# jklebes/MetropolisEngine

Hardware: AMD Instinct MI355X
Metric: MC steps/sec (chains x sweeps) at 2^20 chains, 16 params (higher is better)
Workload: dtype f64

## Files before the change

include/metropolis_engine.h:

```cpp
#ifndef METROPOLIS_ENGINE_H
#define METROPOLIS_ENGINE_H

#include <stddef.h>
#include <stdint.h>

#ifdef __cplusplus
extern "C" {
#endif

#define ME_ABI_VERSION 1

typedef struct me_engine me_engine;

typedef enum me_status {
  ME_OK = 0,
  ME_ERR_INVALID = 1,
  ME_ERR_UNSUPPORTED = 2,
  ME_ERR_HIP = 3,
  ME_ERR_NUMERIC = 4,
  ME_ERR_STATE = 5
} me_status;

typedef enum me_dtype { ME_F32 = 0, ME_F64 = 1 } me_dtype;

// ... 61 lines not shown
  const char *user_energy_name;
} me_config;

int me_abi_version(void);

int me_load_plugin(const char *path);

int me_create(const me_config *config, me_engine **out);
int me_destroy(me_engine *engine);

int me_step(me_engine *engine, int32_t n_sweeps);
typedef enum me_step_kind_t {
  ME_STEP_ALL = 0,
  ME_STEP_REAL_GROUP = 1,
  ME_STEP_COMPLEX_GROUP = 2,
  ME_STEP_COMPLEX_MAGNITUDE_PHASE = 3
} me_step_kind_t;
int me_step_kind(me_engine *engine, int32_t kind, int32_t n_sweeps);
int me_measure(me_engine *engine);
int me_cycle(me_engine *engine, int32_t n_sweeps);
int me_cycle_stats(me_engine *engine, uint64_t *fused_cycles);
int me_set_reject_condition(me_engine *engine, int32_t reject_kind, double reject_bound);
int me_set_energy(me_engine *engine, int32_t energy_kind, const double *energy_coeffs, int32_t n_energy_coeffs,
                  const char *user_energy_name);
int me_step_injected(me_engine *engine, int32_t kind, int32_t n_sweeps, const double *normals, const double *uniforms);

int me_field_components(me_engine *engine, int32_t field, int32_t *n_components);
int me_energy_terms(me_engine *engine, int32_t *n_terms);
int me_get(me_engine *engine, int32_t field, int64_t chain_begin, int64_t n_chains, double *dst);
int me_set(me_engine *engine, int32_t field, int64_t chain_begin, int64_t n_chains, const double *src);
int me_recompute_energy(me_engine *engine);

int me_constants(me_engine *engine, double *alpha, int32_t *m, double *ratio);
int me_counters(me_engine *engine, uint64_t *step_index, uint64_t *measure_step_counter);
int me_set_counters(me_engine *engine, uint64_t step_index, uint64_t measure_step_counter);
int me_accept_stats(me_engine *engine, uint64_t *accepted, uint64_t *proposed);
int me_set_accept_stats(me_engine *engine, uint64_t accepted, uint64_t proposed);

int me_pooled_moments_size(me_engine *engine, int64_t *n_doubles);
int me_pooled_moments_geometry(me_engine *engine, int32_t *matrix_core, int32_t *tile_chains, int32_t *partial_rows);
int me_pooled_moments(me_engine *engine, double *host_out, int64_t n_doubles);
int me_pooled_moments_device(me_engine *engine, void *device_out, int64_t n_doubles);
int me_pooled_moments_begin(me_engine *engine);
int me_pooled_moments_end(me_engine *engine, double *host_out, int64_t n_doubles);
#define ME_COMM_ID_BYTES 128
int me_comm_unique_id(void *id_out, size_t bytes);
int me_comm_init_rank(me_engine *engine, const void *unique_id, size_t bytes, int32_t rank, int32_t world);
int me_comm_destroy(me_engine *engine);
int me_comm_info(me_engine *engine, int32_t *rank, int32_t *world, int32_t *rccl_version);
int me_pooled_moments_allreduce(me_engine *engine, double *host_out, int64_t n_doubles);
int me_pooled_moments_allreduce_begin(me_engine *engine);
int me_set_shared_factor(me_engine *engine, const double *packed_factor, int64_t n_doubles);
int me_set_cache_budget(int64_t bytes);
int me_get_shared_factor(me_engine *engine, double *packed_factor, int64_t n_doubles, int32_t *is_set);

int me_trace_enable(me_engine *engine, int64_t n_traced, int64_t stride);
int me_trace_shape(me_engine *engine, int64_t *rows, int64_t *cols, int64_t *n_traced);
int me_trace_get(me_engine *engine, double *dst, int64_t n_doubles);

int me_sync(me_engine *engine);
int me_set_stream(me_engine *engine, void *hip_stream);
int me_time_steps(me_engine *engine, int32_t n_launches, int32_t n_sweeps, float *elapsed_ms);

int me_set_temperature_ladder(me_engine *engine, const double *temps, int32_t n_rungs);
int me_temperature_ladder(me_engine *engine, double *temps, int32_t capacity, int32_t *n_rungs);
int me_replica_exchange(me_engine *engine, int32_t n_rounds);
int me_replica_stats(me_engine *engine, uint64_t *round, uint64_t *attempted, uint64_t *accepted, int32_t n_pairs);
int me_set_replica_stats(me_engine *engine, uint64_t round, const uint64_t *attempted, const uint64_t *accepted,
                         int32_t n_pairs);
int me_pooled_moments_range(me_engine *engine, int64_t chain_begin, int64_t n_chains, double *host_out, int64_t n_doubles);

int me_set_temperature(me_engine *engine, double temp);
int me_population_resample(me_engine *engine, double new_temp);
int me_population_stats(me_engine *engine, uint64_t *stages, double *stage_temps, double *log_weight, double *neff_fraction,
                        int64_t *n_finite, int64_t capacity);
int me_set_population_stats(me_engine *engine, uint64_t stages, const double *stage_temps, const double *log_weight,
                            const double *neff_fraction, const int64_t *n_finite);
int me_population_families(me_engine *engine, int64_t chain_begin, int64_t n, int64_t *dst);
int me_set_population_families(me_engine *engine, int64_t chain_begin, int64_t n, const int64_t *src);

int me_energy_samples_enable(me_engine *engine, int64_t capacity_records);
int me_energy_samples_record(me_engine *engine);
int me_energy_samples_count(me_engine *engine, int64_t *records, int64_t *capacity);
int me_energy_samples_get(me_engine *engine, int64_t record_begin, int64_t n_records, double *dst);
int me_energy_samples_set(me_engine *engine, int64_t n_records, const double *src);
int me_mbar_solve(me_engine *engine, double tolerance, int32_t max_iterations, double *f_out, int32_t *iterations,
                  double *residual, int64_t *n_used_out);
int me_mbar_solve_newton(me_engine *engine, double tolerance, int32_t max_iterations, double *f_out, int32_t *iterations,
                         double *residual, double *gradient, int32_t *newton_steps, int32_t *fallback_steps, int64_t *n_used_out);
int me_mbar_solve_newton_samples(int32_t device_id, const double *energies, const int32_t *rungs, int64_t n_samples,
                                 const double *ladder_temps, int32_t n_rungs, double tolerance, int32_t max_iterations,
                                 double *f_out, int32_t *iterations, double *residual, double *gradient, int32_t *newton_steps,
                                 int32_t *fallback_steps, int64_t *n_used_out);
int me_mbar_reweight(me_engine *engine, const double *f, const double *temps, int32_t n, double *ln_z, double *mean_e,
                     double *var_e, double *neff_fraction);
int me_mbar_solve_samples(int32_t device_id, const double *energies, const int32_t *rungs, int64_t n_samples,
                          const double *ladder_temps, int32_t n_rungs, double tolerance, int32_t max_iterations, double *f_out,
                          int32_t *iterations, double *residual, int64_t *n_used_out);
int me_mbar_reweight_samples(int32_t device_id, const double *energies, const int32_t *rungs, int64_t n_samples,
                             const double *ladder_temps, int32_t n_rungs, const double *f, const double *temps, int32_t n,
                             double *ln_z, double *mean_e, double *var_e, double *neff_fraction);
int me_mbar_gram(me_engine *engine, const double *f, const double *temps, int32_t n_targets, double *gram,
                 double *column_counts, double *ln_z, double *mean_e, int64_t *n_used);
int me_mbar_gram_samples(int32_t device_id, const double *energies, const int32_t *rungs, int64_t n_samples,
                         const double *ladder_temps, int32_t n_rungs, const double *f, const double *temps, int32_t n_targets,
                         double *gram, double *column_counts, double *ln_z, double *mean_e, int64_t *n_used);
// ... 71 lines not shown
```

metropolisengine_amd/_capi.py:

```python
import ctypes
import os

PKG_DIR = os.path.dirname(os.path.abspath(__file__))
LIB_PATH = os.environ.get("METROPOLIS_HIP_LIB") or os.path.join(PKG_DIR, "lib", "libmetropolis_hip.so")
ABI_VERSION = 1

ME_OK, ME_ERR_INVALID, ME_ERR_UNSUPPORTED, ME_ERR_HIP, ME_ERR_NUMERIC, ME_ERR_STATE = range(6)
ME_F32, ME_F64 = 0, 1
(ENERGY_ISO_QUAD, ENERGY_DIAG_QUAD, ENERGY_DENSE_QUAD, ENERGY_LANDAU_TOY, ENERGY_CYLINDER, ENERGY_USER,
 ENERGY_USER_INDIRECT, ENERGY_LANDAU_TERMS) = range(8)
FLAG_TRACK_COVARIANCE = 1
FLAG_REFERENCE_ENERGY_LEDGERS = 2
REJECT_NONE, REJECT_ABS_REAL0_GE, REJECT_USER = 0, 1, 2
STEP_ALL, STEP_REAL_GROUP, STEP_COMPLEX_GROUP, STEP_COMPLEX_MAGNITUDE_PHASE = range(4)
COV_REFERENCE, COV_FIXED, COV_POOLED = 0, 1, 2
COMM_ID_BYTES = 128
(FIELD_PARAMS, FIELD_ENERGY, FIELD_WIDTH, FIELD_MEAN, FIELD_COV, FIELD_OBS_MEAN, FIELD_FACTOR, FIELD_ENERGY_TOTAL) = range(8)

_dp = ctypes.POINTER(ctypes.c_double)


def double_ptr(arr):
    return arr.ctypes.data_as(_dp)

# ... 15 lines not shown
        ("temp", ctypes.c_double), ("target_acceptance", ctypes.c_double), ("sampling_width", ctypes.c_double),
        ("energy_kind", ctypes.c_int32), ("n_energy_coeffs", ctypes.c_int32), ("energy_coeffs", _dp),
        ("reject_kind", ctypes.c_int32), ("flags", ctypes.c_int32), ("reject_bound", ctypes.c_double),
        ("initial_params", _dp), ("covariance_real", _dp), ("covariance_complex", _dp),
        ("user_energy_name", ctypes.c_char_p),
    ]


_H = ctypes.c_void_p
SYMBOLS = {
    "me_abi_version": (ctypes.c_int, []),
    "me_load_plugin": (ctypes.c_int, [ctypes.c_char_p]),
    "me_create": (ctypes.c_int, [ctypes.POINTER(MeConfig), ctypes.POINTER(_H)]),
    "me_destroy": (ctypes.c_int, [_H]),
    "me_step": (ctypes.c_int, [_H, ctypes.c_int32]),
    "me_measure": (ctypes.c_int, [_H]),
    "me_cycle": (ctypes.c_int, [_H, ctypes.c_int32]),
    "me_cycle_stats": (ctypes.c_int, [_H, ctypes.POINTER(ctypes.c_uint64)]),
    "me_step_kind": (ctypes.c_int, [_H, ctypes.c_int32, ctypes.c_int32]),
    "me_set_reject_condition": (ctypes.c_int, [_H, ctypes.c_int32, ctypes.c_double]),
    "me_set_energy": (ctypes.c_int, [_H, ctypes.c_int32, _dp, ctypes.c_int32, ctypes.c_char_p]),
    "me_step_injected": (ctypes.c_int, [_H, ctypes.c_int32, ctypes.c_int32, _dp, _dp]),
    "me_field_components": (ctypes.c_int, [_H, ctypes.c_int32, ctypes.POINTER(ctypes.c_int32)]),
    "me_energy_terms": (ctypes.c_int, [_H, ctypes.POINTER(ctypes.c_int32)]),
    "me_pooled_moments_begin": (ctypes.c_int, [_H]),
    "me_pooled_moments_end": (ctypes.c_int, [_H, ctypes.POINTER(ctypes.c_double), ctypes.c_int64]),
    "me_detect_equilibration": (ctypes.c_int, [ctypes.c_int32, ctypes.POINTER(ctypes.c_double), ctypes.c_int64,
                                               ctypes.c_int64, ctypes.c_int32, ctypes.c_int32,
                                               ctypes.POINTER(ctypes.c_int64), ctypes.POINTER(ctypes.c_double),
                                               ctypes.POINTER(ctypes.c_double)]),
    "me_get": (ctypes.c_int, [_H, ctypes.c_int32, ctypes.c_int64, ctypes.c_int64, _dp]),
    "me_set": (ctypes.c_int, [_H, ctypes.c_int32, ctypes.c_int64, ctypes.c_int64, _dp]),
    "me_recompute_energy": (ctypes.c_int, [_H]),
    "me_constants": (ctypes.c_int, [_H, _dp, ctypes.POINTER(ctypes.c_int32), _dp]),
    "me_counters": (ctypes.c_int, [_H, ctypes.POINTER(ctypes.c_uint64), ctypes.POINTER(ctypes.c_uint64)]),
    "me_set_counters": (ctypes.c_int, [_H, ctypes.c_uint64, ctypes.c_uint64]),
    "me_accept_stats": (ctypes.c_int, [_H, ctypes.POINTER(ctypes.c_uint64), ctypes.POINTER(ctypes.c_uint64)]),
    "me_pooled_moments_size": (ctypes.c_int, [_H, ctypes.POINTER(ctypes.c_int64)]),
    "me_pooled_moments_geometry": (ctypes.c_int, [_H, ctypes.POINTER(ctypes.c_int32), ctypes.POINTER(ctypes.c_int32),
                                                  ctypes.POINTER(ctypes.c_int32)]),
    "me_pooled_moments": (ctypes.c_int, [_H, _dp, ctypes.c_int64]),
    "me_pooled_moments_device": (ctypes.c_int, [_H, ctypes.c_void_p, ctypes.c_int64]),
    "me_comm_unique_id": (ctypes.c_int, [ctypes.c_void_p, ctypes.c_size_t]),
    "me_comm_init_rank": (ctypes.c_int, [_H, ctypes.c_void_p, ctypes.c_size_t, ctypes.c_int32, ctypes.c_int32]),
    "me_comm_destroy": (ctypes.c_int, [_H]),
    "me_comm_info": (ctypes.c_int, [_H, ctypes.POINTER(ctypes.c_int32), ctypes.POINTER(ctypes.c_int32),
                                    ctypes.POINTER(ctypes.c_int32)]),
    "me_pooled_moments_allreduce": (ctypes.c_int, [_H, _dp, ctypes.c_int64]),
    "me_pooled_moments_allreduce_begin": (ctypes.c_int, [_H]),
    "me_set_shared_factor": (ctypes.c_int, [_H, _dp, ctypes.c_int64]),
    "me_get_shared_factor": (ctypes.c_int, [_H, _dp, ctypes.c_int64, ctypes.POINTER(ctypes.c_int32)]),
    "me_set_accept_stats": (ctypes.c_int, [_H, ctypes.c_uint64, ctypes.c_uint64]),
    "me_set_cache_budget": (ctypes.c_int, [ctypes.c_int64]),
    "me_trace_enable": (ctypes.c_int, [_H, ctypes.c_int64, ctypes.c_int64]),
    "me_trace_shape": (ctypes.c_int, [_H, ctypes.POINTER(ctypes.c_int64), ctypes.POINTER(ctypes.c_int64),
                                      ctypes.POINTER(ctypes.c_int64)]),
    "me_trace_get": (ctypes.c_int, [_H, _dp, ctypes.c_int64]),
    "me_sync": (ctypes.c_int, [_H]),
    "me_set_stream": (ctypes.c_int, [_H, ctypes.c_void_p]),
    "me_time_steps": (ctypes.c_int, [_H, ctypes.c_int32, ctypes.c_int32, ctypes.POINTER(ctypes.c_float)]),
    "me_last_error": (ctypes.c_int, [_H, ctypes.c_char_p, ctypes.c_size_t]),
    "me_supported": (ctypes.c_int, [ctypes.c_int32, ctypes.c_int32, ctypes.c_int32, ctypes.c_int32]),
    "me_set_temperature_ladder": (ctypes.c_int, [_H, _dp, ctypes.c_int32]),
    "me_temperature_ladder": (ctypes.c_int, [_H, _dp, ctypes.c_int32, ctypes.POINTER(ctypes.c_int32)]),
    "me_replica_exchange": (ctypes.c_int, [_H, ctypes.c_int32]),
    "me_replica_stats": (ctypes.c_int, [_H, ctypes.POINTER(ctypes.c_uint64), ctypes.POINTER(ctypes.c_uint64),
                                        ctypes.POINTER(ctypes.c_uint64), ctypes.c_int32]),
    "me_set_replica_stats": (ctypes.c_int, [_H, ctypes.c_uint64, ctypes.POINTER(ctypes.c_uint64),
                                            ctypes.POINTER(ctypes.c_uint64), ctypes.c_int32]),
    "me_pooled_moments_range": (ctypes.c_int, [_H, ctypes.c_int64, ctypes.c_int64, _dp, ctypes.c_int64]),
    "me_set_temperature": (ctypes.c_int, [_H, ctypes.c_double]),
    "me_population_resample": (ctypes.c_int, [_H, ctypes.c_double]),
    "me_population_stats": (ctypes.c_int, [_H, ctypes.POINTER(ctypes.c_uint64), _dp, _dp, _dp, ctypes.POINTER(ctypes.c_int64),
                                           ctypes.c_int64]),
    "me_set_population_stats": (ctypes.c_int, [_H, ctypes.c_uint64, _dp, _dp, _dp, ctypes.POINTER(ctypes.c_int64)]),
    "me_population_families": (ctypes.c_int, [_H, ctypes.c_int64, ctypes.c_int64, ctypes.POINTER(ctypes.c_int64)]),
    "me_set_population_families": (ctypes.c_int, [_H, ctypes.c_int64, ctypes.c_int64, ctypes.POINTER(ctypes.c_int64)]),
    "me_energy_samples_enable": (ctypes.c_int, [_H, ctypes.c_int64]),
    "me_energy_samples_record": (ctypes.c_int, [_H]),
    "me_energy_samples_count": (ctypes.c_int, [_H, ctypes.POINTER(ctypes.c_int64), ctypes.POINTER(ctypes.c_int64)]),
    "me_energy_samples_get": (ctypes.c_int, [_H, ctypes.c_int64, ctypes.c_int64, _dp]),
    "me_energy_samples_set": (ctypes.c_int, [_H, ctypes.c_int64, _dp]),
    "me_mbar_solve": (ctypes.c_int, [_H, ctypes.c_double, ctypes.c_int32, _dp, ctypes.POINTER(ctypes.c_int32), _dp,
                                     ctypes.POINTER(ctypes.c_int64)]),
    "me_mbar_solve_newton": (ctypes.c_int, [_H, ctypes.c_double, ctypes.c_int32, _dp, ctypes.POINTER(ctypes.c_int32), _dp, _dp,
                                            ctypes.POINTER(ctypes.c_int32), ctypes.POINTER(ctypes.c_int32),
                                            ctypes.POINTER(ctypes.c_int64)]),
    "me_mbar_solve_newton_samples": (ctypes.c_int, [ctypes.c_int32, _dp, ctypes.POINTER(ctypes.c_int32), ctypes.c_int64, _dp,
                                                    ctypes.c_int32, ctypes.c_double, ctypes.c_int32, _dp,
                                                    ctypes.POINTER(ctypes.c_int32), _dp, _dp, ctypes.POINTER(ctypes.c_int32),
                                                    ctypes.POINTER(ctypes.c_int32), ctypes.POINTER(ctypes.c_int64)]),
    "me_mbar_reweight": (ctypes.c_int, [_H, _dp, _dp, ctypes.c_int32, _dp, _dp, _dp, _dp]),
    "me_mbar_solve_samples": (ctypes.c_int, [ctypes.c_int32, _dp, ctypes.POINTER(ctypes.c_int32), ctypes.c_int64, _dp,
                                             ctypes.c_int32, ctypes.c_double, ctypes.c_int32, _dp,
                                             ctypes.POINTER(ctypes.c_int32), _dp, ctypes.POINTER(ctypes.c_int64)]),
    "me_mbar_reweight_samples": (ctypes.c_int, [ctypes.c_int32, _dp, ctypes.POINTER(ctypes.c_int32), ctypes.c_int64, _dp,
                                                ctypes.c_int32, _dp, _dp, ctypes.c_int32, _dp, _dp, _dp, _dp]),
    "me_mbar_gram": (ctypes.c_int, [_H, _dp, _dp, ctypes.c_int32, _dp, _dp, _dp, _dp, ctypes.POINTER(ctypes.c_int64)]),
    "me_mbar_gram_samples": (ctypes.c_int, [ctypes.c_int32, _dp, ctypes.POINTER(ctypes.c_int32), ctypes.c_int64, _dp,
                                            ctypes.c_int32, _dp, _dp, ctypes.c_int32, _dp, _dp, _dp, _dp,
                                            ctypes.POINTER(ctypes.c_int64)]),
    "me_mbar_energy_shift": (ctypes.c_int, [_H, _dp]),
    "me_mbar_gram_observables": (ctypes.c_int, [_H, _dp, _dp, ctypes.c_int32, _dp, _dp, _dp, _dp, _dp,
                                                ctypes.POINTER(ctypes.c_int64)]),
    "me_mbar_gram_observables_samples": (ctypes.c_int, [ctypes.c_int32, _dp, ctypes.POINTER(ctypes.c_int32), ctypes.c_int64, _dp,
                                                        ctypes.c_int32, _dp, ctypes.c_int32, _dp, _dp, ctypes.c_int32, _dp, _dp,
# ... 92 lines not shown
```

metropolisengine_amd/csrc/me_api.hip:

```cpp
#include <algorithm>
#include <cmath>
#include <cstdlib>
#include <cstring>
#include <dlfcn.h>
#include <mutex>
#include <memory>
#include <string>
#include <atomic>
#include <chrono>
#include <vector>

#include "me_engine.h"

namespace me {

static std::vector<const KernelSet *> &registry() {
  static std::vector<const KernelSet *> sets;
  return sets;
}
static std::mutex &registry_mutex() {
  static std::mutex m;
  return m;
}
void register_kernel_set(const KernelSet *set) {
// ... 80 lines not shown
static bool initial_shape_is_identity(const me_config *c) {
  if (c->covariance_real)
    for (int i = 0; i < c->n_real; ++i)
      for (int j = 0; j <= i; ++j)
        if (c->covariance_real[i * c->n_real + j] != (i == j ? 1.0 : 0.0)) return false;
  if (c->covariance_complex)
    for (int i = 0; i < c->n_complex; ++i)
      for (int j = 0; j <= i; ++j) {
        const double re = c->covariance_complex[2 * (i * c->n_complex + j)], im = c->covariance_complex[2 * (i * c->n_complex + j) + 1];
        if (re != (i == j ? 1.0 : 0.0) || (i != j && im != 0.0)) return false;
      }
  return true;
}

int fail(me_engine *e, int code, const std::string &msg) {
  if (e) e->err = msg;
  else g_create_error = msg;
  return code;
}

static void to_device_type(const double *src, size_t count, int dtype, std::vector<unsigned char> &out) {
  out.resize(count * (dtype == ME_F32 ? 4 : 8));
  if (dtype == ME_F32) {
    float *o = reinterpret_cast<float *>(out.data());
    for (size_t i = 0; i < count; ++i) o[i] = (float)src[i];
  } else {
    std::memcpy(out.data(), src, count * 8);
  }
}

hipError_t upload(DeviceBuffer &dst, const double *src, size_t count, int dtype) {
  std::vector<unsigned char> bytes;
  to_device_type(src, count, dtype, bytes);
  const hipError_t err = dst.resize(bytes.size());
  return err != hipSuccess ? err : hipMemcpy(dst.get(), bytes.data(), bytes.size(), hipMemcpyHostToDevice);
}

int refuse_stale_total(me_engine *e, const char *subject) {
  if (!e->stale_total) return ME_OK;
  return fail(e, ME_ERR_UNSUPPORTED, std::string(subject) + " not available with ME_FLAG_REFERENCE_ENERGY_LEDGERS: its two ledgers "
                                                            "make the energy of a chain ambiguous");
}

static int report_status(me_engine *e, unsigned int bits) {
  if (!bits) return ME_OK;
  ME_HIP(e, hipMemsetAsync(e->status.get(), 0, sizeof(unsigned int), e->stream));
  std::string msg = "numeric failure in at least one chain:";
  if (bits & ST_NONFINITE_ENERGY) msg += " non-finite energy;";
  if (bits & ST_BAD_PIVOT) msg += " non-positive Cholesky pivot (proposal covariance not positive definite);";
  if (bits & ST_BAD_WIDTH) msg += " sampling width <= 0;";
  return fail(e, ME_ERR_NUMERIC, msg);
}
int check_status(me_engine *e) {
  unsigned long long *scratch = e->host_scratch.get<unsigned long long>();
  ME_HIP(e, hipMemcpyAsync(&scratch[0], e->status.get(), sizeof(unsigned int), hipMemcpyDeviceToHost, e->stream));
  ME_HIP(e, hipStreamSynchronize(e->stream));
  return report_status(e, (unsigned int)scratch[0]);
}

}

using namespace me;

namespace {

int broadcast(me_engine *e, DeviceBuffer &dst, const std::vector<double> &row, bool tiled = false) {
  std::vector<unsigned char> bytes;
  to_device_type(row.data(), row.size(), e->dtype, bytes);
  ME_HIP(e, hipMemcpyAsync(e->row_dev.get(), bytes.data(), bytes.size(), hipMemcpyHostToDevice, e->stream));
  if (tiled) ME_HIP(e, launch_broadcast_tiled(dst.get(), e->row_dev.get(), (int)row.size(), e->n, e->dtype, e->stream));
  else ME_HIP(e, launch_broadcast_rows(dst.get(), e->row_dev.get(), (int)row.size(), e->n, e->dtype, e->stream));
  ME_HIP(e, hipStreamSynchronize(e->stream));
  return ME_OK;
}

template <typename T>
void gather_rows(const T *t, int comps, int64_t n_chains, double *dst) {
  for (int r = 0; r < comps; ++r)
    for (int64_t c = 0; c < n_chains; ++c) dst[c * comps + r] = (double)t[(size_t)r * n_chains + c];
}
template <typename T>
void scatter_rows(T *t, int comps, int64_t n_chains, const double *src) {
  for (int r = 0; r < comps; ++r)
    for (int64_t c = 0; c < n_chains; ++c) t[(size_t)r * n_chains + c] = (T)src[c * comps + r];
}
template <typename T>
void transpose_tiled(T *t, int entries, int64_t tile0, int64_t chain_begin, int64_t n_chains, double *dst, const double *src) {
  const size_t tile_values = (size_t)entries * 64;
  auto at = [&](int64_t c, int k) { return (size_t)((c >> 6) - tile0) * tile_values + (size_t)k * 64 + (size_t)(c & 63); };
  for (int64_t i = 0; i < n_chains; ++i)
    for (int k = 0; k < entries; ++k) {
      if (dst) dst[i * entries + k] = (double)t[at(chain_begin + i, k)];
      else t[at(chain_begin + i, k)] = (T)src[i * entries + k];
    }
}

int copy_tiled(me_engine *e, void *field_ptr, int entries, int64_t chain_begin, int64_t n_chains, double *dst, const double *src) {
  const int64_t tile0 = chain_begin >> 6, tile1 = (chain_begin + n_chains - 1) >> 6;
  const size_t tile_values = (size_t)entries * 64, n_values = (size_t)(tile1 - tile0 + 1) * tile_values;
  unsigned char *dev = (unsigned char *)field_ptr + (size_t)tile0 * tile_values * e->esize;
  std::vector<unsigned char> tmp(n_values * e->esize);
  const bool whole = (chain_begin & 63) == 0 && (((chain_begin + n_chains) & 63) == 0 || chain_begin + n_chains == e->n);
  if (dst || !whole) {
    ME_HIP(e, hipMemcpyAsync(tmp.data(), dev, tmp.size(), hipMemcpyDeviceToHost, e->stream));
    ME_HIP(e, hipStreamSynchronize(e->stream));
  }
  if (e->dtype == ME_F32) transpose_tiled(reinterpret_cast<float *>(tmp.data()), entries, tile0, chain_begin, n_chains, dst, src);
  else transpose_tiled(reinterpret_cast<double *>(tmp.data()), entries, tile0, chain_begin, n_chains, dst, src);
  if (src) {
    ME_HIP(e, hipMemcpyAsync(dev, tmp.data(), tmp.size(), hipMemcpyHostToDevice, e->stream));
    ME_HIP(e, hipStreamSynchronize(e->stream));
  }
  return dst ? check_status(e) : ME_OK;
}

int field_info(me_engine *e, int field, void **ptr, int *comps) {
  switch (field) {
    case ME_FIELD_PARAMS: *ptr = e->x.get(); *comps = e->d; return ME_OK;
    case ME_FIELD_ENERGY: *ptr = e->energy.get(); *comps = e->n_terms; return ME_OK;
    case ME_FIELD_WIDTH: *ptr = e->width.get(); *comps = e->width_rows; return ME_OK;
    case ME_FIELD_MEAN: *ptr = e->mean.get(); *comps = e->d; return ME_OK;
    case ME_FIELD_OBS_MEAN: *ptr = e->obs_mean.get(); *comps = e->nobs; return ME_OK;
    case ME_FIELD_COV:
      if (!e->cov)
        return fail(e, ME_ERR_UNSUPPORTED, "this engine keeps no per-chain covariance: for large parameter spaces it is "
                                           "kept on request only (me_config.flags: ME_FLAG_TRACK_COVARIANCE), and not "
                                           "at all where the field would pass 4 GiB");
      *ptr = e->cov.get(); *comps = e->p; return ME_OK;
    case ME_FIELD_ENERGY_TOTAL:
      if (!e->stale_total)
        return fail(e, ME_ERR_UNSUPPORTED, "this engine keeps one coherent energy ledger (sum ME_FIELD_ENERGY); a separate "
                                           "energy_total exists with ME_FLAG_REFERENCE_ENERGY_LEDGERS only");
      *ptr = e->energy.get<unsigned char>() + (size_t)e->n_terms * (size_t)e->n * e->esize; *comps = 1; return ME_OK;
    case ME_FIELD_FACTOR:
      if (!e->factor) return fail(e, ME_ERR_UNSUPPORTED, "this engine keeps no per-chain proposal factors (dimensions "
                                                         "without per-chain kernels, or a field beyond 4 GiB)");
      *ptr = e->factor.get(); *comps = e->p; return ME_OK;
    default: return fail(e, ME_ERR_INVALID, "unknown field id");
  }
}

int upload_shared_factor(me_engine *e, const double *packed) {
  ME_HIP(e, upload(e->shared_factor, packed, (size_t)e->p, e->dtype));
  if (e->shared_full) {
    std::vector<double> full((size_t)e->nr * e->nr, 0.0);
    for (int i = 0; i < e->nr; ++i)
      for (int j = 0; j <= i; ++j) full[(size_t)i * e->nr + j] = packed[i * (i + 1) / 2 + j];
    ME_HIP(e, upload(e->shared_full, full.data(), full.size(), e->dtype));
    if (e->shared_image) ME_HIP(e, e->ks->prepare_matrix(e->shared_full.get(), e->shared_image.get(), e->stream));
  }
  return ME_OK;
}

void fill_step_launch(me_engine *e, StepLaunch &l, int n_sweeps) {
  l.n_real = e->nr;
  l.n_complex = e->nc;
  l.x = e->x.get();
  l.energy = e->energy.get();
  l.width = e->width.get();
  l.factor = e->cov_kind == CK_PER_CHAIN ? e->factor.get() : e->shared_factor.get();
  l.factor_full = e->shared_full.get();
  l.factor_image = e->shared_image.get();
  l.energy_image = e->energy_image.get();
  l.coef_device = e->coef_dev.get();
  l.coef_host = e->coef.data();
  l.n_coef = (int)e->coef.size();
  l.inj_normals = nullptr;
  l.inj_uniforms = nullptr;
  l.group = GROUP_ALL;
  l.split_widths = (e->width_rows == 3 && !e->widths_synced) ? 1 : 0;
  l.stale_total = e->stale_total ? 1 : 0;
  l.cov = e->cov.get();
  l.accept_slots = e->accept_slots.get<unsigned long long>();
  l.status = e->status.get<unsigned int>();
  l.n = e->n;
  l.chain_offset = e->chain_offset;
  l.step_index = e->step_index;
  l.seed = e->seed;
  l.n_sweeps = n_sweeps;
  l.energy_kind = e->energy_kind;
  l.cov_kind = e->cov_kind;
  l.reject_kind = e->reject_kind;
  l.grid_blocks = e->grid_blocks;
  l.reject_bound = e->reject_bound;
  l.temp = e->temp;
  l.ratio = e->ratio;
  l.target_acceptance = e->target_acceptance;
  l.damping = std::max((double)e->measure_count / (double)e->m, 200.0);
  l.ladder = e->ladder.n_rungs ? e->ladder.table.get() : nullptr;
  l.tiles_per_rung = e->ladder.n_rungs ? (int)(e->n / (64ll * e->ladder.n_rungs)) : 0;
}

int check_reject_kind(me_engine *e, int reject_kind, int energy_kind, int n_real) {
  if (reject_kind < ME_REJECT_NONE || reject_kind > ME_REJECT_USER) return fail(e, ME_ERR_INVALID, "unknown reject_kind");
  if (reject_kind == ME_REJECT_USER && !is_user_kind(energy_kind))
    return fail(e, ME_ERR_INVALID, "ME_REJECT_USER needs a user-energy plugin (it supplies me_user_reject)");
  if (reject_kind == ME_REJECT_ABS_REAL0_GE && n_real == 0)
    return fail(e, ME_ERR_INVALID, "ME_REJECT_ABS_REAL0_GE needs a real parameter");
  return ME_OK;
}
int check_user_reject(me_engine *e, int reject_kind, const KernelSet *ks) {
  if (reject_kind == ME_REJECT_USER && !ks->has_user_reject)
    return fail(e, ME_ERR_UNSUPPORTED,
                "ME_REJECT_USER: this user-energy plugin defines no me_user_reject (#define ME_USER_HAS_REJECT in its source)");
  return ME_OK;
}

}

namespace me {
namespace {
std::atomic<long long> g_cache_budget{224ll << 20};
}
long long cache_budget_bytes() { return g_cache_budget.load(std::memory_order_relaxed); }
void set_cache_budget_bytes(long long bytes) { g_cache_budget.store(bytes, std::memory_order_relaxed); }
}


int me_set_cache_budget(int64_t bytes) {
  if (bytes < 0) return fail(nullptr, ME_ERR_INVALID, "cache budget must be >= 0");
  me::set_cache_budget_bytes(bytes);
  return ME_OK;
}

int me_abi_version(void) { return ME_ABI_VERSION; }

int me_supported(int32_t dtype, int32_t n_real, int32_t n_complex, int32_t energy_kind) {
  return find_kernel_set(dtype, n_real, n_complex, energy_kind, nullptr) ? 1 : 0;
}

namespace {

int validate_config(const me_config *c, const KernelSet **ks_out) {
  if (c->abi_version != ME_ABI_VERSION) return fail(nullptr, ME_ERR_INVALID, "me_config.abi_version mismatch");
  if (c->n_real < 0 || c->n_complex < 0 || c->n_real + c->n_complex == 0)
    return fail(nullptr, ME_ERR_INVALID,
                "must give at least one real or complex parameter (metropolis_engine.py:37-39)");
  if (c->n_chains <= 0) return fail(nullptr, ME_ERR_INVALID, "n_chains must be positive");
  if (!(c->temp >= 0)) return fail(nullptr, ME_ERR_INVALID, "temp must be >= 0 (metropolis_engine.py:92)");
  if (!(c->target_acceptance > 0 && c->target_acceptance < 1))
    return fail(nullptr, ME_ERR_INVALID, "target_acceptance must be in (0, 1)");
  if (!(c->sampling_width > 0)) return fail(nullptr, ME_ERR_INVALID, "sampling_width must be > 0");
  if (c->dtype != ME_F32 && c->dtype != ME_F64) return fail(nullptr, ME_ERR_INVALID, "unknown dtype");
// ... 71 lines not shown
                  "engines or use ME_COV_FIXED / ME_COV_POOLED");
    l.keep_per_chain = false;
  }
  const long long rows = std::max<long long>(c->n_real + 2 * c->n_complex, 2 * c->n_real + c->n_complex);
  if (rows * padded * esz >= limit)
    return fail(nullptr, ME_ERR_UNSUPPORTED,
                "a per-chain field would exceed 4 GiB on this engine; shard the chains over more engines");
  l.keep_cov = l.keep_per_chain ||
               ((!ks->per_chain_cov || ks->streams_packed) && ks->tracks_cov && (c->flags & ME_FLAG_TRACK_COVARIANCE));
  l.x_tiled = ks->tiled_state;
  l.width_rows = (c->n_real > 0 && c->n_complex > 0) ? 3 : 1;
  return ME_OK;
}

std::unique_ptr<me_engine> configure(const me_config *c, const KernelSet *ks, const Layout &l) {
  std::unique_ptr<me_engine> e(new me_engine);
  e->device = c->device_id;
  e->ks = ks;
  e->n_terms = ks->energy_terms(c->energy_kind);
  e->dtype = c->dtype;
  e->esize = c->dtype == ME_F32 ? 4 : 8;
  e->n = c->n_chains;
  e->nr = c->n_real;
  e->nc = c->n_complex;
  e->d = e->nr + 2 * e->nc;
  e->p = packed_total(e->nr, e->nc);
  e->nobs = n_observables(e->nr, e->nc);
  e->chain_offset = c->chain_offset;
  e->seed = c->seed;
  e->temp = c->temp;
  e->target_acceptance = c->target_acceptance;
  e->energy_kind = c->energy_kind;
  e->reject_kind = c->reject_kind;
  e->reject_bound = c->reject_bound;
  e->cov_mode = c->cov_mode;
  e->coef.assign(c->energy_coeffs, c->energy_coeffs + c->n_energy_coeffs);
  e->alpha = -norm_ppf(c->target_acceptance / 2.0);
  e->m = e->nr + e->nc;
  e->ratio = (1.0 - 1.0 / e->m) * std::sqrt(2.0 * M_PI) * std::exp(e->alpha * e->alpha / 2.0) / 2.0 * e->alpha +
             1.0 / (e->m * c->target_acceptance * (1.0 - c->target_acceptance));
  if (const char *g = std::getenv("ME_GRID_BLOCKS")) e->grid_blocks = std::atoi(g);
  e->x_tiled = l.x_tiled;
  e->stale_total = (c->flags & ME_FLAG_REFERENCE_ENERGY_LEDGERS) != 0;
  e->width_rows = l.width_rows;
  e->n_slots = (e->n + 31) / 32 + 8;
  return e;
}

int allocate(me_engine *e, const Layout &l) {
  const KernelSet *ks = e->ks;
  ME_HIP(e, hipSetDevice(e->device));
  ME_HIP(e, e->stream.create());
  const size_t n = (size_t)e->n, tiles = (size_t)padded_chains(e->n), es = e->esize;
  ME_HIP(e, e->x.resize((e->x_tiled ? tiles : n) * e->d * es));
  ME_HIP(e, e->energy.resize(n * (e->n_terms + (e->stale_total ? 1 : 0)) * es));
  ME_HIP(e, e->width.resize(n * e->width_rows * es));
  ME_HIP(e, e->mean.resize(n * e->d * es));
  ME_HIP(e, e->obs_mean.resize(n * e->nobs * es));
  if (l.keep_cov) ME_HIP(e, e->cov.resize(tiles * e->p * es));
  if (l.keep_per_chain) ME_HIP(e, e->factor.resize(tiles * e->p * es));
  ME_HIP(e, e->shared_factor.resize((size_t)e->p * es));
  if (e->nc == 0) ME_HIP(e, e->shared_full.resize((size_t)e->nr * e->nr * es));
  if (e->shared_full && ks->prepare_matrix) ME_HIP(e, e->shared_image.resize(ks->matrix_image_bytes));
  ME_HIP(e, e->row_dev.resize((size_t)std::max(std::max(e->d, e->p), e->nobs) * es));
  ME_HIP(e, e->accept_slots.resize((size_t)e->n_slots * sizeof(unsigned long long)));
  ME_HIP(e, e->accept_total.resize(sizeof(unsigned long long)));
  ME_HIP(e, e->status.resize(sizeof(unsigned int)));
  const size_t moments_bytes = sizeof(double) * (size_t)moments_size(e->nr, e->nc);
  ME_HIP(e, e->pool.dev.resize(moments_bytes));
  ME_HIP(e, e->host_scratch.allocate(64));
  e->host_scratch.get<unsigned long long>()[0] = e->host_scratch.get<unsigned long long>()[1] = 0;
  ME_HIP(e, e->pool.host.allocate(moments_bytes));
  if (pool_reduce_supported(e->nr, e->nc, e->dtype))
    ME_HIP(e, e->pool.partials.resize(sizeof(double) * (size_t)pool_reduce_blocks(e->n, e->nr, e->nc) *
                                      (size_t)(1 + e->d + e->nr + e->nc + e->d * (e->d + 1) / 2)));
  ME_HIP(e, hipMemsetAsync(e->accept_slots.get(), 0, e->accept_slots.bytes(), e->stream));
  ME_HIP(e, hipMemsetAsync(e->status.get(), 0, sizeof(unsigned int), e->stream));
  return ME_OK;
}

int upload_coefficients(me_engine *e) {
  const std::vector<double> &coef = e->coef;
  const bool runtime_dims = e->ks->n_real < 0;
  std::vector<double> form;
  if (runtime_dims && e->energy_kind == ME_ENERGY_DIAG_QUAD) {
    if ((int)coef.size() != e->nr + e->nc) return fail(e, ME_ERR_INVALID, "wrong number of energy coefficients for this energy kind");
    form.assign(coef.begin(), coef.end());
    form.insert(form.end(), coef.begin() + e->nr, coef.end());
  } else if (runtime_dims && e->energy_kind == ME_ENERGY_DENSE_QUAD) {
    if ((int)coef.size() != e->d * e->d) return fail(e, ME_ERR_INVALID, "wrong number of energy coefficients for this energy kind");
    form.reserve((size_t)e->d * (e->d + 1) / 2);
    for (int i = 0; i < e->d; ++i)
      for (int j = 0; j <= i; ++j)
        form.push_back(i == j ? coef[(size_t)i * e->d + i] : coef[(size_t)i * e->d + j] + coef[(size_t)j * e->d + i]);
  } else if (e->energy_kind == ME_ENERGY_DENSE_QUAD || (is_user_kind(e->energy_kind) && !coef.empty())) {
    form = coef;
  } else {
    return ME_OK;
  }
  ME_HIP(e, upload(e->coef_dev, form.data(), form.size(), e->dtype));
  if (!runtime_dims && e->energy_kind == ME_ENERGY_DENSE_QUAD && e->ks->prepare_matrix) {
    ME_HIP(e, e->energy_image.resize(e->ks->matrix_image_bytes));
    ME_HIP(e, e->ks->prepare_matrix(e->coef_dev.get(), e->energy_image.get(), e->stream));
  }
  return ME_OK;
}

int initial_state(me_engine *e, const me_config *c) {
  std::vector<double> init(c->initial_params, c->initial_params + e->d);
  std::vector<double> obs(e->nobs);
  for (int i = 0; i < e->nr; ++i) {
    obs[i] = std::fabs(init[i]);
    obs[e->nr + e->nc + i] = init[i] * init[i];
  }
  for (int j = 0; j < e->nc; ++j) obs[e->nr + j] = std::hypot(init[e->nr + j], init[e->nr + e->nc + j]);
  const int pr = packed_real(e->nr);
  std::vector<double> c0(e->p, 0.0);
  bool identity = true;
  for (int i = 0; i < e->nr; ++i)
    for (int j = 0; j <= i; ++j) {
      const double v = c->covariance_real ? c->covariance_real[i * e->nr + j] : (i == j ? 1.0 : 0.0);
      c0[i * (i + 1) / 2 + j] = v;
      identity = identity && v == (i == j ? 1.0 : 0.0);
    }
  for (int i = 0; i < e->nc; ++i) {
    for (int j = 0; j < i; ++j) {
      const double re = c->covariance_complex ? c->covariance_complex[2 * (i * e->nc + j)] : 0.0;
      const double im = c->covariance_complex ? c->covariance_complex[2 * (i * e->nc + j) + 1] : 0.0;
      c0[pr + i * i + 2 * j] = re;
      c0[pr + i * i + 2 * j + 1] = im;
      identity = identity && re == 0.0 && im == 0.0;
    }
    const double dg = c->covariance_complex ? c->covariance_complex[2 * (i * e->nc + i)] : 1.0;
    c0[pr + i * i + 2 * i] = dg;
    identity = identity && dg == 1.0;
  }
  std::vector<double> f0 = c0;
  for (int i = 0; i < e->nc; ++i)
    for (int j = 0; j < i; ++j) f0[pr + i * i + 2 * j + 1] = -f0[pr + i * i + 2 * j + 1];
  if (!host_factor(f0, e->nr, e->nc))
    return fail(e, ME_ERR_INVALID, "initial covariance matrix is not positive definite (metropolis_engine.py:270)");
  int rc = ME_OK;
  std::vector<double> width_row((size_t)e->width_rows, c->sampling_width);
  if ((rc = broadcast(e, e->x, init, e->x_tiled)) || (rc = broadcast(e, e->mean, init)) || (rc = broadcast(e, e->obs_mean, obs)) ||
      (rc = broadcast(e, e->width, width_row)) || (e->cov && (rc = broadcast(e, e->cov, c0, true))) ||
      (e->factor && (rc = broadcast(e, e->factor, f0, true))) || (rc = upload_shared_factor(e, f0.data())))
    return rc;
  e->cov_kind = identity ? CK_IDENTITY : (e->ks->n_real < 0 && e->factor) ? CK_PER_CHAIN : CK_SHARED;
  return ME_OK;
}

int initial_energy(me_engine *e) {
  const int rc = me_recompute_energy(e);
  if (rc != ME_OK) return rc;
  const hipError_t herr = hipStreamSynchronize(e->stream);
  if (herr != hipSuccess) return fail(e, ME_ERR_HIP, std::string("initial energy evaluation: ") + hipGetErrorString(herr));
  return ME_OK;
}

}

int me_create(const me_config *c, me_engine **out) {
  if (!c || !out) return fail(nullptr, ME_ERR_INVALID, "null config or output pointer");
  *out = nullptr;
  const KernelSet *ks = nullptr;
  Layout layout;
  int rc;
  if ((rc = validate_config(c, &ks)) || (rc = decide_layout(c, ks, layout))) return rc;
  int n_dev = 0;
  if (hipGetDeviceCount(&n_dev) != hipSuccess || n_dev <= 0)
    return fail(nullptr, ME_ERR_HIP, "no HIP device available (this library has no CPU fallback)");
  if (c->device_id < 0 || c->device_id >= n_dev) return fail(nullptr, ME_ERR_INVALID, "device_id out of range");

  std::unique_ptr<me_engine> e = configure(c, ks, layout);
  if ((rc = allocate(e.get(), layout)) || (rc = upload_coefficients(e.get())) || (rc = initial_state(e.get(), c)) ||
      (rc = initial_energy(e.get())))
    return fail(nullptr, rc, e->err);
  *out = e.release();
  return ME_OK;
}

int me_set_reject_condition(me_engine *e, int32_t reject_kind, double reject_bound) {
  if (!e) return ME_ERR_INVALID;
  int rc;
  if ((rc = check_reject_kind(e, reject_kind, e->energy_kind, e->nr)) || (rc = check_user_reject(e, reject_kind, e->ks))) return rc;
  e->reject_kind = reject_kind;
  e->reject_bound = reject_bound;
  return ME_OK;
}

int me_set_energy(me_engine *e, int32_t energy_kind, const double *coeffs, int32_t n_coeffs, const char *user_name) {
  if (!e) return ME_ERR_INVALID;
  if (n_coeffs < 0 || (n_coeffs > 0 && !coeffs)) return fail(e, ME_ERR_INVALID, "energy coefficients missing");
  if (e->ks->n_real < 0) return fail(e, ME_ERR_UNSUPPORTED, "me_set_energy: not available on the runtime-dimension kernel set");
  if (energy_kind == ME_ENERGY_DENSE_QUAD)
    return fail(e, ME_ERR_UNSUPPORTED, "me_set_energy: the dense quadratic form keeps device images of its matrix; create a new engine");
  const KernelSet *ks = find_kernel_set(e->dtype, e->nr, e->nc, energy_kind, user_name);
// ... 1 lines not shown
    return fail(e, ME_ERR_UNSUPPORTED, is_user_kind(energy_kind)
                    ? std::string("no user-energy plugin named '") + (user_name ? user_name : "") + "' is loaded for these dimensions"
                    : "energy kind " + std::to_string(energy_kind) + " is not compiled for these dimensions");
  if (ks->tiled_state != e->ks->tiled_state || ks->per_chain_cov != e->ks->per_chain_cov || ks->streams_packed != e->ks->streams_packed ||
      ks->tracks_cov != e->ks->tracks_cov)
    return fail(e, ME_ERR_UNSUPPORTED, "me_set_energy: the plugin was built with other per-chain covariance options than this engine's kernel set");
  if (e->reject_kind == ME_REJECT_USER && !ks->has_user_reject)
    return fail(e, ME_ERR_UNSUPPORTED, "me_set_energy: the engine's wall is the plugin's me_user_reject, which the new energy does not define");
  const int n_terms = ks->energy_terms(energy_kind);
  ME_HIP(e, hipSetDevice(e->device));
  ME_HIP(e, hipStreamSynchronize(e->stream));
  DeviceBuffer ledger, coef_dev;
  if (n_terms != e->n_terms)
    ME_HIP(e, ledger.resize((size_t)e->n * (size_t)(n_terms + (e->stale_total ? 1 : 0)) * e->esize));
  if (is_user_kind(energy_kind) && n_coeffs > 0) ME_HIP(e, upload(coef_dev, coeffs, (size_t)n_coeffs, e->dtype));
  if (n_terms != e->n_terms) {
    e->energy = std::move(ledger);
    e->n_terms = n_terms;
    if (e->trace.chains > 0) e->trace.restart();
  }
  e->coef.assign(coeffs, coeffs + n_coeffs);
  e->coef_dev = std::move(coef_dev);
  e->ks = ks;
  e->energy_kind = energy_kind;
  const int rc = me_recompute_energy(e);
  if (rc != ME_OK) return rc;
  ME_HIP(e, hipStreamSynchronize(e->stream));
  return check_status(e);
}

int me_load_plugin(const char *path) {
  if (!path) return fail(nullptr, ME_ERR_INVALID, "null plugin path");
  void *handle = dlopen(path, RTLD_NOW | RTLD_GLOBAL);
  if (!handle) return fail(nullptr, ME_ERR_INVALID, std::string("dlopen failed: ") + dlerror());
  return ME_OK;
}

int me_destroy(me_engine *e) {
  if (!e) return ME_ERR_INVALID;
  (void)hipSetDevice(e->device);
  if (e->stream) (void)hipStreamSynchronize(e->stream);
  if (e->pool.copy_stream) (void)hipStreamSynchronize(e->pool.copy_stream);
  delete e;
  return ME_OK;
}

int me_recompute_energy(me_engine *e) {
  if (!e) return ME_ERR_INVALID;
  ME_HIP(e, hipSetDevice(e->device));
  EnergyLaunch l;
  l.n_real = e->nr;
  l.n_complex = e->nc;
  l.total_row = e->stale_total ? e->n_terms : -1;
  l.x = e->x.get();
  l.energy = e->energy.get();
  l.coef_device = e->coef_dev.get();
  l.coef_host = e->coef.data();
  l.n_coef = (int)e->coef.size();
  l.status = e->status.get<unsigned int>();
  l.n = e->n;
  l.energy_kind = e->energy_kind;
  l.grid_blocks = e->grid_blocks;
  hipError_t err = e->ks->init_energy(l, e->stream);
  if (err == hipErrorInvalidValue) return fail(e, ME_ERR_INVALID, "wrong number of energy coefficients for this energy kind");
  ME_HIP(e, err);
  return ME_OK;
}

static int split_widths(me_engine *e) {
  if (e->width_rows != 3 || !e->widths_synced) return ME_OK;
  const size_t row = (size_t)e->n * e->esize;
  for (int r = 1; r <= 2; ++r)
    ME_HIP(e, hipMemcpyAsync(e->width.get<unsigned char>() + r * row, e->width.get(), row, hipMemcpyDeviceToDevice, e->stream));
  e->widths_synced = false;
  return ME_OK;
}

static int resolve_step_kind(me_engine *e, int kind, int *group, bool *magphase) {
  *magphase = false;
  *group = GROUP_ALL;
  const bool mixed = e->nr > 0 && e->nc > 0;
  switch (kind) {
    case ME_STEP_ALL: return ME_OK;
    case ME_STEP_REAL_GROUP:
      if (e->nr == 0) return fail(e, ME_ERR_INVALID, "this engine has no real parameters");
      *group = mixed ? GROUP_REAL : GROUP_ALL;
      return ME_OK;
    case ME_STEP_COMPLEX_GROUP:
      if (e->nc == 0) return fail(e, ME_ERR_INVALID, "this engine has no complex parameters");
      *group = mixed ? GROUP_COMPLEX : GROUP_ALL;
      return ME_OK;
    case ME_STEP_COMPLEX_MAGNITUDE_PHASE:
      if (e->nc == 0) return fail(e, ME_ERR_INVALID, "this engine has no complex parameters");
      if (!e->ks->magphase || !e->cov)
        return fail(e, ME_ERR_UNSUPPORTED, "the magnitude-phase sampler needs the per-chain covariance kernels");
      *magphase = true;
      return ME_OK;
    default: return fail(e, ME_ERR_INVALID, "unknown step kind");
  }
}

static void count_steps(me_engine *e, int n_sweeps, int group = GROUP_ALL, bool magphase = false) {
  if (group == GROUP_ALL && !magphase) e->widths_synced = true;
  e->step_index += (unsigned long long)n_sweeps;
  e->proposed += (unsigned long long)e->n * (unsigned long long)n_sweeps * (magphase ? 2ull : 1ull);
}

static int launch_step_kind(me_engine *e, int kind, int n_sweeps, const void *inj_normals, const void *inj_uniforms) {
  int group;
  bool magphase;
  int rc = resolve_step_kind(e, kind, &group, &magphase);
  if (rc != ME_OK) return rc;
  if ((group != GROUP_ALL || magphase) && (rc = split_widths(e)) != ME_OK) return rc;
  StepLaunch l;
  fill_step_launch(e, l, n_sweeps);
  l.group = group;
  l.inj_normals = inj_normals;
  l.inj_uniforms = inj_uniforms;
  hipError_t err = magphase ? e->ks->magphase(l, e->stream) : e->ks->step(l, e->stream);
  if (err == hipErrorNotSupported) return fail(e, ME_ERR_UNSUPPORTED, "this step kind is not compiled for this engine");
  ME_HIP(e, err);
  count_steps(e, n_sweeps, group, magphase);
  return ME_OK;
}

int me_step(me_engine *e, int32_t n_sweeps) { return me_step_kind(e, ME_STEP_ALL, n_sweeps); }

int me_step_kind(me_engine *e, int32_t kind, int32_t n_sweeps) {
  if (!e) return ME_ERR_INVALID;
  if (n_sweeps <= 0) return fail(e, ME_ERR_INVALID, "n_sweeps must be positive");
  ME_HIP(e, hipSetDevice(e->device));
  return launch_step_kind(e, kind, n_sweeps, nullptr, nullptr);
}

int me_step_injected(me_engine *e, int32_t kind, int32_t n_sweeps, const double *normals, const double *uniforms) {
  if (!e || !normals || !uniforms) return ME_ERR_INVALID;
  if (n_sweeps <= 0) return fail(e, ME_ERR_INVALID, "n_sweeps must be positive");
  if (e->dtype != ME_F64) return fail(e, ME_ERR_UNSUPPORTED, "injected-stream replay is compiled for float64 engines only");
  ME_HIP(e, hipSetDevice(e->device));
  const bool magphase = kind == ME_STEP_COMPLEX_MAGNITUDE_PHASE;
  const size_t n = (size_t)e->n, k = (size_t)n_sweeps;
  const size_t nz = magphase ? (size_t)e->nc : (size_t)e->d, nu = magphase ? (size_t)e->nc + 2 : 1;
  std::vector<double> zn(k * nz * n), un(k * nu * n);
  for (size_t s = 0; s < k; ++s)
    for (size_t c = 0; c < n; ++c) {
      for (size_t j = 0; j < nz; ++j) zn[(s * nz + j) * n + c] = normals[(s * n + c) * nz + j];
      for (size_t j = 0; j < nu; ++j) un[(s * nu + j) * n + c] = uniforms[(s * n + c) * nu + j];
    }
  DeviceBuffer zd, ud;
  ME_HIP(e, zd.resize(zn.size() * sizeof(double)));
  if (ud.resize(un.size() * sizeof(double)) != hipSuccess) return fail(e, ME_ERR_HIP, "hipMalloc of the injected uniforms failed");
  if (hipMemcpy(zd.get(), zn.data(), zd.bytes(), hipMemcpyHostToDevice) != hipSuccess ||
      hipMemcpy(ud.get(), un.data(), ud.bytes(), hipMemcpyHostToDevice) != hipSuccess)
    return fail(e, ME_ERR_HIP, "upload of the injected streams failed");
  int rc = launch_step_kind(e, kind, n_sweeps, zd.get(), ud.get());
  if (rc == ME_OK && hipStreamSynchronize(e->stream) != hipSuccess) rc = fail(e, ME_ERR_HIP, "injected step failed");
  return rc;
}

namespace {
void fill_measure_launch(me_engine *e, MeasureLaunch &l, unsigned long long count) {
  l.n_real = e->nr;
  l.n_complex = e->nc;
  l.x = e->x.get();
  l.width = e->width.get();
  l.mean = e->mean.get();
  l.cov = e->cov.get();
  l.obs_mean = e->obs_mean.get();
  l.factor = e->factor.get();
  l.status = e->status.get<unsigned int>();
  l.n = e->n;
  l.measure_count = count;
  l.update_cov = (count > 50 && e->cov) ? 1 : 0;
  l.split_widths = (e->width_rows == 3 && !e->widths_synced) ? 1 : 0;
  l.write_factor = (l.update_cov && e->cov_mode == ME_COV_REFERENCE) ? 1 : 0;
  l.grid_blocks = e->grid_blocks;
}

int commit_measure(me_engine *e, const MeasureLaunch &l) {
  e->measure_count = l.measure_count;
  if (l.write_factor) e->cov_kind = CK_PER_CHAIN;
  if (e->trace.chains > 0) {
    const long long cols = e->d + e->n_terms + e->width_rows;
    if (e->trace.rows == e->trace.capacity) {
      const long long cap = e->trace.capacity ? 2 * e->trace.capacity : 1024;
      DeviceBuffer bigger;
      ME_HIP(e, bigger.resize(sizeof(double) * (size_t)(cap * cols * e->trace.chains)));
      if (e->trace.dev) {
        ME_HIP(e, hipMemcpyAsync(bigger.get(), e->trace.dev.get(), sizeof(double) * (size_t)(e->trace.rows * cols * e->trace.chains),
                                 hipMemcpyDeviceToDevice, e->stream));
        ME_HIP(e, hipStreamSynchronize(e->stream));
      }
      e->trace.dev = std::move(bigger);
      e->trace.capacity = cap;
    }
    const int rows_valid = (e->width_rows == 3 && e->widths_synced) ? 1 : e->width_rows;
    double *row = e->trace.dev.get<double>() + e->trace.rows * cols * e->trace.chains;
    ME_HIP(e, launch_trace(e->x.get(), e->energy.get(), e->width.get(), e->n, e->d, e->n_terms, rows_valid, e->dtype, e->trace.chains,
                           e->trace.stride, row, e->stream, e->x_tiled));
    if (rows_valid != e->width_rows) {
      double *widths = row + (size_t)(e->d + e->n_terms) * e->trace.chains;
      for (int r = 1; r < 3; ++r)
        ME_HIP(e, hipMemcpyAsync(widths + (size_t)r * e->trace.chains, widths, sizeof(double) * (size_t)e->trace.chains,
                                 hipMemcpyDeviceToDevice, e->stream));
    }
    e->trace.rows += 1;
  }
  return ME_OK;
}
}

int me_measure(me_engine *e) {
  if (!e) return ME_ERR_INVALID;
  ME_HIP(e, hipSetDevice(e->device));
  MeasureLaunch l;
  fill_measure_launch(e, l, e->measure_count + 1);
  ME_HIP(e, e->ks->measure(l, e->stream));
  return commit_measure(e, l);
}

int me_cycle(me_engine *e, int32_t n_sweeps) {
  if (!e) return ME_ERR_INVALID;
  if (n_sweeps <= 0) return fail(e, ME_ERR_INVALID, "n_sweeps must be positive");
  ME_HIP(e, hipSetDevice(e->device));
  if (e->ks->cycle) {
    StepLaunch sl;
    fill_step_launch(e, sl, n_sweeps);
    MeasureLaunch ml;
    fill_measure_launch(e, ml, e->measure_count + 1);
    ml.split_widths = 0;
    const hipError_t err = e->ks->cycle(sl, ml, e->stream);
    if (err == hipSuccess) {
      count_steps(e, n_sweeps);
      e->fused_cycles += 1;
      return commit_measure(e, ml);
    }
    if (err != hipErrorNotSupported) ME_HIP(e, err);
    (void)hipGetLastError();
  }
  const int rc = me_step(e, n_sweeps);
  return rc != ME_OK ? rc : me_measure(e);
}

int me_cycle_stats(me_engine *e, uint64_t *fused_cycles) {
  if (!e || !fused_cycles) return ME_ERR_INVALID;
  *fused_cycles = e->fused_cycles;
  return ME_OK;
}

int me_trace_enable(me_engine *e, int64_t n_traced, int64_t stride) {
  if (!e) return ME_ERR_INVALID;
  if (n_traced < 0 || stride < 1 || (n_traced > 0 && (n_traced - 1) * stride >= e->n))
    return fail(e, ME_ERR_INVALID, "traced chains out of range");
  ME_HIP(e, hipSetDevice(e->device));
  ME_HIP(e, hipStreamSynchronize(e->stream));
  e->trace.restart();
  e->trace.chains = n_traced;
  e->trace.stride = stride;
  return ME_OK;
}

int me_trace_shape(me_engine *e, int64_t *rows, int64_t *cols, int64_t *n_traced) {
  if (!e) return ME_ERR_INVALID;
  if (rows) *rows = e->trace.rows;
  if (cols) *cols = e->d + e->n_terms + e->width_rows;
  if (n_traced) *n_traced = e->trace.chains;
  return ME_OK;
}

int me_trace_get(me_engine *e, double *dst, int64_t n_doubles) {
  if (!e || !dst) return ME_ERR_INVALID;
  const long long want = e->trace.rows * (e->d + e->n_terms + e->width_rows) * e->trace.chains;
  if (n_doubles != want) return fail(e, ME_ERR_INVALID, "wrong trace buffer length");
  if (want == 0) return ME_OK;
  ME_HIP(e, hipSetDevice(e->device));
  ME_HIP(e, hipStreamSynchronize(e->stream));
  ME_HIP(e, hipMemcpy(dst, e->trace.dev.get(), sizeof(double) * (size_t)want, hipMemcpyDeviceToHost));
  return ME_OK;
}

int me_field_components(me_engine *e, int32_t field, int32_t *n_components) {
  if (!e || !n_components) return ME_ERR_INVALID;
  void *ptr;
  int comps;
  int rc = field_info(e, field, &ptr, &comps);
  if (rc == ME_OK) *n_components = comps;
  return rc;
}

int me_energy_terms(me_engine *e, int32_t *n_terms) {
  if (!e || !n_terms) return ME_ERR_INVALID;
  *n_terms = e->n_terms;
  return ME_OK;
}

int me_get(me_engine *e, int32_t field, int64_t chain_begin, int64_t n_chains, double *dst) {
  if (!e || !dst) return ME_ERR_INVALID;
  if (chain_begin < 0 || n_chains < 0 || chain_begin + n_chains > e->n) return fail(e, ME_ERR_INVALID, "chain range out of bounds");
  ME_HIP(e, hipSetDevice(e->device));
  void *ptr;
  int comps;
  int rc = field_info(e, field, &ptr, &comps);
  if (rc != ME_OK) return rc;
  if (n_chains == 0) return ME_OK;
  if (field == ME_FIELD_COV || field == ME_FIELD_FACTOR || (field == ME_FIELD_PARAMS && e->x_tiled))
    return copy_tiled(e, ptr, comps, chain_begin, n_chains, dst, nullptr);
  std::vector<unsigned char> tmp((size_t)comps * n_chains * e->esize);
  for (int r = 0; r < comps; ++r)
    ME_HIP(e, hipMemcpyAsync(tmp.data() + (size_t)r * n_chains * e->esize,
                             (const unsigned char *)ptr + ((size_t)r * e->n + chain_begin) * e->esize,
                             (size_t)n_chains * e->esize, hipMemcpyDeviceToHost, e->stream));
  ME_HIP(e, hipStreamSynchronize(e->stream));
  if (e->dtype == ME_F32) gather_rows(reinterpret_cast<const float *>(tmp.data()), comps, n_chains, dst);
  else gather_rows(reinterpret_cast<const double *>(tmp.data()), comps, n_chains, dst);
  if (field == ME_FIELD_WIDTH && e->width_rows == 3 && e->widths_synced)
    for (int64_t c = 0; c < n_chains; ++c) dst[c * 3 + 1] = dst[c * 3 + 2] = dst[c * 3];
  return check_status(e);
}

int me_set(me_engine *e, int32_t field, int64_t chain_begin, int64_t n_chains, const double *src) {
  if (!e || !src) return ME_ERR_INVALID;
  if (chain_begin < 0 || n_chains < 0 || chain_begin + n_chains > e->n) return fail(e, ME_ERR_INVALID, "chain range out of bounds");
  ME_HIP(e, hipSetDevice(e->device));
  void *ptr;
  int comps;
  int rc = field_info(e, field, &ptr, &comps);
  if (rc != ME_OK) return rc;
  if (field == ME_FIELD_WIDTH && e->width_rows == 3 && (chain_begin != 0 || n_chains != e->n))
    return fail(e, ME_ERR_INVALID, "widths of a mixed engine must be set for all chains at once");
  if (n_chains == 0) return ME_OK;
  if (field == ME_FIELD_COV || field == ME_FIELD_FACTOR || (field == ME_FIELD_PARAMS && e->x_tiled)) {
    rc = copy_tiled(e, ptr, comps, chain_begin, n_chains, nullptr, src);
    if (rc != ME_OK) return rc;
    if (field == ME_FIELD_FACTOR) e->cov_kind = CK_PER_CHAIN;
    return ME_OK;
  }
  std::vector<unsigned char> tmp((size_t)comps * n_chains * e->esize);
  if (e->dtype == ME_F32) scatter_rows(reinterpret_cast<float *>(tmp.data()), comps, n_chains, src);
  else scatter_rows(reinterpret_cast<double *>(tmp.data()), comps, n_chains, src);
  for (int r = 0; r < comps; ++r)
    ME_HIP(e, hipMemcpyAsync((unsigned char *)ptr + ((size_t)r * e->n + chain_begin) * e->esize,
                             tmp.data() + (size_t)r * n_chains * e->esize, (size_t)n_chains * e->esize,
                             hipMemcpyHostToDevice, e->stream));
  ME_HIP(e, hipStreamSynchronize(e->stream));
  if (field == ME_FIELD_FACTOR) e->cov_kind = CK_PER_CHAIN;
  if (field == ME_FIELD_WIDTH && e->width_rows == 3) e->widths_synced = false;
  return ME_OK;
}

int me_constants(me_engine *e, double *alpha, int32_t *m, double *ratio) {
  if (!e) return ME_ERR_INVALID;
  if (alpha) *alpha = e->alpha;
  if (m) *m = e->m;
  if (ratio) *ratio = e->ratio;
  return ME_OK;
}

int me_counters(me_engine *e, uint64_t *step_index, uint64_t *measure_step_counter) {
  if (!e) return ME_ERR_INVALID;
  if (step_index) *step_index = e->step_index;
  if (measure_step_counter) *measure_step_counter = e->measure_count;
  return ME_OK;
}

int me_set_counters(me_engine *e, uint64_t step_index, uint64_t measure_step_counter) {
  if (!e) return ME_ERR_INVALID;
  if (measure_step_counter < 1) return fail(e, ME_ERR_INVALID, "measure_step_counter starts at 1");
  e->step_index = step_index;
  e->measure_count = measure_step_counter;
  return ME_OK;
}

int me_accept_stats(me_engine *e, uint64_t *accepted, uint64_t *proposed) {
  if (!e) return ME_ERR_INVALID;
  ME_HIP(e, hipSetDevice(e->device));
  unsigned long long *scratch = e->host_scratch.get<unsigned long long>();
  ME_HIP(e, launch_sum_slots(e->accept_slots.get<unsigned long long>(), e->n_slots, e->accept_total.get<unsigned long long>(), e->stream));
  ME_HIP(e, hipMemcpyAsync(&scratch[1], e->accept_total.get(), sizeof(unsigned long long), hipMemcpyDeviceToHost, e->stream));
  ME_HIP(e, hipMemcpyAsync(&scratch[0], e->status.get(), sizeof(unsigned int), hipMemcpyDeviceToHost, e->stream));
  ME_HIP(e, hipStreamSynchronize(e->stream));
  if (accepted) *accepted = scratch[1];
  if (proposed) *proposed = e->proposed;
  return report_status(e, (unsigned int)scratch[0]);
// ... 10 lines not shown
  e->proposed = proposed;
  return ME_OK;
}

int me_pooled_moments_size(me_engine *e, int64_t *n_doubles) {
  if (!e || !n_doubles) return ME_ERR_INVALID;
  *n_doubles = moments_size(e->nr, e->nc);
  return ME_OK;
}

int me_pooled_moments_geometry(me_engine *e, int32_t *matrix_core, int32_t *tile_chains, int32_t *partial_rows) {
  if (!e || !matrix_core || !tile_chains || !partial_rows) return ME_ERR_INVALID;
  if (!e->pool.partials) return fail(e, ME_ERR_UNSUPPORTED, "pooled moments: dimension too large for the reduction kernel");
  *matrix_core = e->ks->pool_stage1 ? 1 : 0;
  *tile_chains = e->ks->pool_stage1 ? 64 : pool_tile_chains(e->nr, e->nc, e->dtype);
  *partial_rows = pool_reduce_blocks(e->n, e->nr, e->nc);
  return ME_OK;
}

namespace {
hipError_t wait_polling(hipEvent_t ev) {
  const auto t0 = std::chrono::steady_clock::now();
  for (;;) {
    const hipError_t rc = hipEventQuery(ev);
    if (rc != hipErrorNotReady) return rc;
    if (std::chrono::steady_clock::now() - t0 > std::chrono::milliseconds(2)) return hipEventSynchronize(ev);
  }
}
hipError_t wait_polling(hipStream_t stream) {
  const auto t0 = std::chrono::steady_clock::now();
  for (;;) {
    const hipError_t rc = hipStreamQuery(stream);
    if (rc != hipErrorNotReady) return rc;
    if (std::chrono::steady_clock::now() - t0 > std::chrono::milliseconds(2)) return hipStreamSynchronize(stream);
  }
}

int check_pooled(me_engine *e, int64_t n_doubles) {
  if (n_doubles != moments_size(e->nr, e->nc)) return fail(e, ME_ERR_INVALID, "wrong pooled-moment buffer length");
  if (e->pool.pending) return fail(e, ME_ERR_STATE, "a pooled-moment reduction is in flight (me_pooled_moments_end first)");
  if (!e->pool.partials) return fail(e, ME_ERR_UNSUPPORTED, "pooled moments: dimension too large for the reduction kernel");
  ME_HIP(e, hipSetDevice(e->device));
  return ME_OK;
}
int enqueue_pool_reduce(me_engine *e, const void *x, long long n_chains, long long n_slots, double proposed, double *device_out) {
  hipError_t err = launch_pool_reduce(x, n_chains, e->nr, e->nc, e->dtype, e->accept_slots.get<unsigned long long>(), n_slots, proposed,
                                      e->pool.partials.get<double>(), device_out, e->stream, e->ks->pool_stage1, e->x_tiled);
  if (err == hipErrorInvalidValue) return fail(e, ME_ERR_UNSUPPORTED, "pooled moments: dimension too large for the reduction kernel");
  ME_HIP(e, err);
  return ME_OK;
}
int enqueue_pooled_moments(me_engine *e, double *device_out, int64_t n_doubles) {
  const int rc = check_pooled(e, n_doubles);
  return rc != ME_OK ? rc : enqueue_pool_reduce(e, e->x.get(), e->n, e->n_slots, (double)e->proposed, device_out);
}
int fetch_pooled_moments(me_engine *e, double *host_out, int64_t n_doubles) {
  const size_t bytes = sizeof(double) * (size_t)n_doubles;
  ME_HIP(e, hipMemcpyAsync(e->pool.host.get<double>(), e->pool.dev.get(), bytes, hipMemcpyDeviceToHost, e->stream));
  ME_HIP(e, wait_polling(e->stream));
  std::memcpy(host_out, e->pool.host.get<double>(), bytes);
  return ME_OK;
}
}

int me_pooled_moments_device(me_engine *e, void *device_out, int64_t n_doubles) {
  if (!e || !device_out) return ME_ERR_INVALID;
  int rc = enqueue_pooled_moments(e, (double *)device_out, n_doubles);
  if (rc != ME_OK) return rc;
  ME_HIP(e, wait_polling(e->stream));
  return ME_OK;
}

int me_pooled_moments(me_engine *e, double *host_out, int64_t n_doubles) {
  if (!e || !host_out) return ME_ERR_INVALID;
  const int rc = enqueue_pooled_moments(e, e->pool.dev.get<double>(), n_doubles);
  return rc != ME_OK ? rc : fetch_pooled_moments(e, host_out, n_doubles);
}

int me_pooled_moments_range(me_engine *e, int64_t chain_begin, int64_t n_chains, double *host_out, int64_t n_doubles) {
  if (!e || !host_out) return ME_ERR_INVALID;
  if (chain_begin < 0 || n_chains <= 0 || chain_begin + n_chains > e->n || chain_begin % 64 != 0 || n_chains % 64 != 0)
    return fail(e, ME_ERR_INVALID, "the chain range must be whole 64-chain tiles inside the engine");
  int rc = check_pooled(e, n_doubles);
  if (rc != ME_OK) return rc;
  const unsigned char *x = e->x.get<unsigned char>();
  if (e->x_tiled) {
    x += (size_t)chain_begin * e->d * e->esize;
  } else {
    const size_t row = (size_t)n_chains * e->esize;
    if (row * e->d > e->pool.range_x.bytes()) {
      ME_HIP(e, hipStreamSynchronize(e->stream));
      ME_HIP(e, e->pool.range_x.reserve(row * e->d));
    }
    ME_HIP(e, hipMemcpy2DAsync(e->pool.range_x.get(), row, x + (size_t)chain_begin * e->esize, (size_t)e->n * e->esize, row, (size_t)e->d,
                               hipMemcpyDeviceToDevice, e->stream));
    x = e->pool.range_x.get<unsigned char>();
  }
  if ((rc = enqueue_pool_reduce(e, x, n_chains, 0, 0.0, e->pool.dev.get<double>())) != ME_OK) return rc;
  return fetch_pooled_moments(e, host_out, n_doubles);
}

namespace {
int begin_pooled(me_engine *e, bool allreduce) {
  if (e->pool.pending) return fail(e, ME_ERR_STATE, "a pooled-moment reduction is already in flight: call me_pooled_moments_end first");
  if (allreduce && !e->comm)
    return fail(e, ME_ERR_STATE, "this engine has no communicator: call me_comm_init_rank first (single-GPU engines use me_pooled_moments)");
  ME_HIP(e, hipSetDevice(e->device));
  if (!e->pool.copy_stream) {
    ME_HIP(e, e->pool.copy_stream.create());
    ME_HIP(e, e->pool.reduced.create(hipEventDisableTiming));
    ME_HIP(e, e->pool.copied.create(hipEventDisableTiming));
  }
  const int64_t n_doubles = moments_size(e->nr, e->nc);
  int rc = enqueue_pooled_moments(e, e->pool.dev.get<double>(), n_doubles);
  if (rc != ME_OK) return rc;
  ME_HIP(e, hipEventRecord(e->pool.reduced, e->stream));
  ME_HIP(e, hipStreamWaitEvent(e->pool.copy_stream, e->pool.reduced, 0));
  if (allreduce) {
    const ncclResult_t nrc = e->rccl->all_reduce(e->pool.dev.get<double>(), e->pool.dev.get<double>(), (size_t)n_doubles, ncclDouble, ncclSum, e->comm, e->pool.copy_stream);
    if (nrc != ncclSuccess) return fail(e, ME_ERR_HIP, std::string("ncclAllReduce: ") + e->rccl->error_string(nrc));
  }
  ME_HIP(e, hipMemcpyAsync(e->pool.host.get<double>(), e->pool.dev.get<double>(), sizeof(double) * (size_t)n_doubles, hipMemcpyDeviceToHost, e->pool.copy_stream));
  ME_HIP(e, hipEventRecord(e->pool.copied, e->pool.copy_stream));
  e->pool.pending = true;
  return ME_OK;
}
}

int me_pooled_moments_begin(me_engine *e) {
  if (!e) return ME_ERR_INVALID;
  return begin_pooled(e, false);
}

int me_pooled_moments_allreduce_begin(me_engine *e) {
  if (!e) return ME_ERR_INVALID;
  return begin_pooled(e, true);
}

// ... 63 lines not shown
    *rccl_version = v;
  }
  return ME_OK;
}

int me_pooled_moments_end(me_engine *e, double *host_out, int64_t n_doubles) {
  if (!e || !host_out) return ME_ERR_INVALID;
  if (!e->pool.pending) return fail(e, ME_ERR_STATE, "no pooled-moment reduction in flight: call me_pooled_moments_begin first");
  if (n_doubles != moments_size(e->nr, e->nc)) return fail(e, ME_ERR_INVALID, "wrong pooled-moment buffer length");
  ME_HIP(e, hipSetDevice(e->device));
  ME_HIP(e, wait_polling(e->pool.copied));
  e->pool.pending = false;
  std::memcpy(host_out, e->pool.host.get<double>(), sizeof(double) * (size_t)n_doubles);
  return ME_OK;
}

int me_set_shared_factor(me_engine *e, const double *packed_factor, int64_t n_doubles) {
  if (!e || !packed_factor) return ME_ERR_INVALID;
  if (e->cov_mode != ME_COV_POOLED) return fail(e, ME_ERR_STATE, "me_set_shared_factor needs cov_mode = ME_COV_POOLED");
  if (n_doubles != e->p) return fail(e, ME_ERR_INVALID, "wrong packed factor length");
  ME_HIP(e, hipSetDevice(e->device));
  ME_HIP(e, hipStreamSynchronize(e->stream));
  int rc = upload_shared_factor(e, packed_factor);
  if (rc != ME_OK) return rc;
  e->cov_kind = CK_SHARED;
  e->shared_host.assign(packed_factor, packed_factor + n_doubles);
  return ME_OK;
}

int me_get_shared_factor(me_engine *e, double *packed_factor, int64_t n_doubles, int32_t *is_set) {
  if (!e || !is_set) return ME_ERR_INVALID;
  *is_set = e->shared_host.empty() ? 0 : 1;
  if (!*is_set) return ME_OK;
  if (!packed_factor || n_doubles != e->p) return fail(e, ME_ERR_INVALID, "wrong packed factor length");
  std::copy(e->shared_host.begin(), e->shared_host.end(), packed_factor);
  return ME_OK;
}

int me_sync(me_engine *e) {
  if (!e) return ME_ERR_INVALID;
  ME_HIP(e, hipSetDevice(e->device));
  ME_HIP(e, hipStreamSynchronize(e->stream));
  return check_status(e);
}

int me_set_stream(me_engine *e, void *hip_stream) {
  if (!e) return ME_ERR_INVALID;
  ME_HIP(e, hipSetDevice(e->device));
  ME_HIP(e, hipStreamSynchronize(e->stream));
  e->stream.lend((hipStream_t)hip_stream);
  return ME_OK;
}

int me_time_steps(me_engine *e, int32_t n_launches, int32_t n_sweeps, float *elapsed_ms) {
  if (!e || !elapsed_ms) return ME_ERR_INVALID;
  if (n_launches <= 0 || n_sweeps <= 0) return fail(e, ME_ERR_INVALID, "n_launches and n_sweeps must be positive");
  ME_HIP(e, hipSetDevice(e->device));
  if (!e->time_start) {
    ME_HIP(e, e->time_start.create());
    ME_HIP(e, e->time_stop.create());
  }
  hipEvent_t start = e->time_start, stop = e->time_stop;
  ME_HIP(e, hipEventRecord(start, e->stream));
  for (int i = 0; i < n_launches; ++i) {
    StepLaunch l;
    fill_step_launch(e, l, n_sweeps);
    hipError_t err = e->ks->step(l, e->stream);
    if (err != hipSuccess) return fail(e, ME_ERR_HIP, std::string("step launch: ") + hipGetErrorString(err));
    count_steps(e, n_sweeps);
  }
  ME_HIP(e, hipEventRecord(stop, e->stream));
  ME_HIP(e, hipEventSynchronize(stop));
  ME_HIP(e, hipEventElapsedTime(elapsed_ms, start, stop));
  return ME_OK;
}

int me_last_error(me_engine *e, char *buf, size_t buf_bytes) {
  if (!buf || buf_bytes == 0) return ME_ERR_INVALID;
  const std::string &s = e ? e->err : g_create_error;
  const size_t k = std::min(buf_bytes - 1, s.size());
  std::memcpy(buf, s.data(), k);
  buf[k] = 0;
  return ME_OK;
}
```

metropolisengine_amd/csrc/me_device.h:

```cpp
#pragma once

#include <type_traits>
#include <utility>

#include <hip/hip_runtime.h>
#include <stdint.h>

#include "me_internal.h"
#include "me_math64.h"

namespace me {

struct U4 {
  uint32_t x, y, z, w;
};

__device__ __forceinline__ uint32_t xor3(uint32_t a, uint32_t b, uint32_t c) {
  return __builtin_amdgcn_bitop3_b32(a, b, c, 0x96);
}
__device__ __forceinline__ U4 philox4x32_10(U4 c, uint32_t k0, uint32_t k1) {
#pragma unroll
  for (int r = 0; r < 10; ++r) {
    const uint64_t p0 = (uint64_t)0xD2511F53u * c.x;
    const uint64_t p1 = (uint64_t)0xCD9E8D57u * c.z;
    U4 n;
    n.x = xor3((uint32_t)(p1 >> 32), c.y, k0);
    n.y = (uint32_t)p1;
    n.z = xor3((uint32_t)(p0 >> 32), c.w, k1);
    n.w = (uint32_t)p0;
    c = n;
    k0 += 0x9E3779B9u;
    k1 += 0xBB67AE85u;
  }
  return c;
}
__device__ __forceinline__ U4 philox_counter(unsigned long long gid, unsigned long long step, int b) {
  U4 ctr;
  ctr.x = (uint32_t)gid;
  ctr.y = (uint32_t)(gid >> 32);
  ctr.z = (uint32_t)step;
  ctr.w = ((uint32_t)(step >> 32) << 16) | (uint32_t)b;
  return ctr;
}
__device__ __forceinline__ U4 philox_block(unsigned long long gid, unsigned long long step, int b, uint32_t seed_lo, uint32_t seed_hi) {
  return philox4x32_10(philox_counter(gid, step, b), seed_lo, seed_hi);
}

__device__ __forceinline__ float fma_(float a, float b, float c) { return __builtin_fmaf(a, b, c); }
__device__ __forceinline__ double fma_(double a, double b, double c) { return __builtin_fma(a, b, c); }

template <typename R>
struct Num;

template <>
struct Num<float> {
  static __device__ __forceinline__ void prepare() {}
  static __device__ __forceinline__ float unit(uint32_t w) {
    return __builtin_fmaf((float)w, 2.3283064365386963e-10f, 1.1641532182693481e-10f);
  }
  static __device__ __forceinline__ void normal_pair(uint32_t wa, uint32_t wb, float &g0, float &g1) {
    const float u1 = unit(wa), u2 = unit(wb);
    const float r = __builtin_amdgcn_sqrtf(-1.3862943611198906f * __builtin_amdgcn_logf(u1));
// ... 793 lines not shown
        static_for<NC>([&](auto row_index) {
          constexpr int i = decltype(row_index)::value;
          R are = 0, aim = 0;
          static_for<i>([&](auto col_index) {
            constexpr int j = decltype(col_index)::value;
            const R lre = use(std::integral_constant<int, cre(NR * (NR + 1) / 2, i, j)>{});
            const R lim = use(std::integral_constant<int, cim(NR * (NR + 1) / 2, i, j)>{});
            const R wre = g[NR + j] * R(0.70710678118654752440), wim = g[NR + NC + j] * R(0.70710678118654752440);
            are += lre * wre - lim * wim;
            aim += lre * wim + lim * wre;
          });
          const R ld = use(std::integral_constant<int, cdiag(NR * (NR + 1) / 2, i)>{});
          are += ld * (g[NR + i] * R(0.70710678118654752440));
          aim += ld * (g[NR + NC + i] * R(0.70710678118654752440));
          if constexpr (GROUP != GROUP_REAL) {
            xp[NR + i] = x[NR + i] + w_c * are;
            xp[NR + NC + i] = x[NR + NC + i] + w_c * aim;
          }
        });
        bool rejected = false;
        if (a.reject_kind == ME_REJECT_ABS_REAL0_GE) rejected = !(N_::abs_(xp[0]) < a.reject_bound);
        else if (a.reject_kind == ME_REJECT_USER) rejected = energy_reject(en, xp, 0);
        R terms_new[Ledger::T];
        const R e_new = ledger.propose(en, xp, terms_new);
        const R diff = e_new - (stale_total ? total_q5 : ledger.partial());
        bool accept = diff <= R(0);
        if constexpr (LADDER) accept = accept || uphill_at<true>(a, c, u_accept, diff);
        else if (a.temp > R(0)) accept = accept || N_::uphill(u_accept, diff, a.inv_temp, a.inv_temp_log2e);
        accept = accept && !rejected;
        bad_energy |= (!rejected && !N_::finite(e_new));
#pragma unroll
        for (int d = 0; d < D; ++d) x[d] = accept ? xp[d] : x[d];
        if (stale_total) total_q5 = accept ? e_new : total_q5;
        else ledger.commit(accept, terms_new);
        w = N_::adapt(w, accept, a.ratio, a.p, a.damping, a.up, a.down);
        if constexpr (GROUP == GROUP_ALL) w_r = w_c = w;
        else if constexpr (GROUP == GROUP_REAL) w_r = w;
        else w_c = w;
        wave_accepted += (unsigned int)__popcll(__ballot(accept));
      }
    } else {
      run_sweeps<R, NR, NC, Energy, CK, INJECT, GROUP, LADDER>(a, en, c, gid, stale_total, x, ledger, total_q5, w, w_r, w_c, fac, wave_accepted, bad_energy);
    }
    bad_width |= !(w > R(0));
#pragma unroll
    for (int d = 0; d < D; ++d) fx.store(d, xoff, x[d]);
    if (stale_total) fe.store(Ledger::T, coff, total_q5);
    else ledger.store(fe, coff);
    fw.store(MIXED ? GROUP : 0, coff, w);
  }
  publish_step(a, blockDim.x >> 6, wave_accepted, bad_energy, bad_width);
}

template <typename R, int NR, int NC, class Energy>
__global__ void __launch_bounds__(kStepThreads) k_init_energy(const R *xs, R *energy, long long n, unsigned int *status,
                                                                Energy en, int total_row) {
  constexpr int D = NR + 2 * NC;
  energy_prepare(en, 0);
  const long long stride = (long long)gridDim.x * kStepThreads;
  for (long long c = (long long)blockIdx.x * kStepThreads + threadIdx.x; c < n; c += stride) {
    R x[D];
#pragma unroll
    for (int d = 0; d < D; ++d) x[d] = xs[state_index<R, D>(c, d, n)];
    constexpr int T = term_count<Energy>::value;
    bool finite = true;
    R total = R(0);
#pragma unroll
    for (int t = 0; t < T; ++t) {
      R e;
      if constexpr (T == 1) e = en(x);
      else e = en.term(t, x);
      energy[(long long)t * n + c] = e;
      total = t == 0 ? e : total + e;
      finite = finite && Num<R>::finite(e);
    }
    if (total_row >= 0) energy[(long long)total_row * n + c] = total;
    if (!finite) atomicOr(status, (unsigned int)ST_NONFINITE_ENERGY);
  }
}

}
#include "me_packed_walk.h"
namespace me {

template <typename R>
struct MeasureArgs {
  const R *x, *width;
  R *mean, *cov, *obs_mean, *factor;
  unsigned int *status;
  long long n;
  R keep;
  R inv_i;
  R cov_keep;
  int update_cov, write_factor, split_widths;
};

template <typename R>
MeasureArgs<R> typed_measure(const MeasureLaunch &l) {
  MeasureArgs<R> a;
  a.x = (const R *)l.x;
  a.width = (const R *)l.width;
  a.mean = (R *)l.mean;
  a.cov = (R *)l.cov;
  a.obs_mean = (R *)l.obs_mean;
  a.factor = (R *)l.factor;
  a.status = l.status;
// ... 288 lines not shown
```

metropolisengine_amd/csrc/me_engine.h:

```cpp
#pragma once

#include <string>
#include <utility>
#include <vector>

#include "me_comm.h"
#include "me_internal.h"

#pragma GCC visibility push(hidden)

namespace me {


class DeviceBuffer {
 public:
  DeviceBuffer() = default;
  DeviceBuffer(DeviceBuffer &&o) noexcept : ptr_(std::exchange(o.ptr_, nullptr)), bytes_(std::exchange(o.bytes_, 0)) {}
  DeviceBuffer &operator=(DeviceBuffer &&o) noexcept {
    if (this != &o) {
      reset();
      ptr_ = std::exchange(o.ptr_, nullptr);
      bytes_ = std::exchange(o.bytes_, 0);
    }
    return *this;
  }
  ~DeviceBuffer() { reset(); }
  void reset() {
    if (ptr_) (void)hipFree(ptr_);
    ptr_ = nullptr;
    bytes_ = 0;
  }
  hipError_t resize(size_t bytes) {
    if (bytes == bytes_) return hipSuccess;
    reset();
    if (bytes == 0) return hipSuccess;
    const hipError_t err = hipMalloc(&ptr_, bytes);
    if (err == hipSuccess) bytes_ = bytes;
    else ptr_ = nullptr;
    return err;
  }
  hipError_t reserve(size_t bytes) { return bytes <= bytes_ ? hipSuccess : resize(bytes); }
  template <typename T = void>
  T *get() const { return static_cast<T *>(ptr_); }
  size_t bytes() const { return bytes_; }
  explicit operator bool() const { return ptr_ != nullptr; }

 private:
  void *ptr_ = nullptr;
  size_t bytes_ = 0;
};

class PinnedBuffer {
 public:
  PinnedBuffer() = default;
  PinnedBuffer(const PinnedBuffer &) = delete;
  PinnedBuffer &operator=(const PinnedBuffer &) = delete;
  ~PinnedBuffer() { reset(); }
  void reset() {
    if (ptr_) (void)hipHostFree(ptr_);
    ptr_ = nullptr;
// ... 25 lines not shown
    if (owned_ && stream_) (void)hipStreamDestroy(stream_);
    stream_ = theirs;
    owned_ = false;
  }
  operator hipStream_t() const { return stream_; }

 private:
  hipStream_t stream_ = nullptr;
  bool owned_ = false;
};

class Event {
 public:
  Event() = default;
  Event(const Event &) = delete;
  Event &operator=(const Event &) = delete;
  ~Event() { reset(); }
  void reset() {
    if (event_) (void)hipEventDestroy(event_);
    event_ = nullptr;
  }
  hipError_t create(unsigned flags = hipEventDefault) {
    reset();
    return hipEventCreateWithFlags(&event_, flags);
  }
  operator hipEvent_t() const { return event_; }

 private:
  hipEvent_t event_ = nullptr;
};

}

struct me_engine {
  int device = 0;
  me::Stream stream;
  const me::KernelSet *ks = nullptr;
  int dtype = ME_F32;
  size_t esize = 4;
  long long n = 0;
  int nr = 0, nc = 0, d = 0, p = 0, nobs = 0;
  unsigned long long chain_offset = 0, seed = 0;
  double temp = 0, target_acceptance = 0.3, alpha = 0, ratio = 0, reject_bound = 0;
  int m = 0, energy_kind = 0, reject_kind = 0, cov_mode = 0;
  bool stale_total = false;
  me::Event time_start, time_stop;
  std::vector<double> shared_host;
  int cov_kind = me::CK_IDENTITY;
  int grid_blocks = 0;
  int n_terms = 1;
  std::vector<double> coef;
  unsigned long long step_index = 0, measure_count = 1;
  unsigned long long fused_cycles = 0;
  me::DeviceBuffer x, energy, width, mean, cov, obs_mean;
  me::DeviceBuffer factor, shared_factor, shared_full, shared_image, energy_image, coef_dev, row_dev;
  me::DeviceBuffer accept_slots, accept_total;
  long long n_slots = 0;
  unsigned long long proposed = 0;
  bool x_tiled = false;
  int width_rows = 1;
  bool widths_synced = true;
  me::DeviceBuffer status;
  me::PinnedBuffer host_scratch;
  struct Pool {
    me::DeviceBuffer dev, partials;
    me::PinnedBuffer host;
    me::DeviceBuffer range_x;
    me::Stream copy_stream;
    me::Event reduced, copied;
    bool pending = false;
  } pool;
  const me::RcclApi *rccl = nullptr;
  ncclComm_t comm = nullptr;
  int comm_rank = 0, comm_world = 1;
  struct Trace {
    me::DeviceBuffer dev;
    long long chains = 0, stride = 1, rows = 0, capacity = 0;
    void restart() {
      dev.reset();
      rows = capacity = 0;
    }
  } trace;
  struct Ladder {
    int n_rungs = 0;
    std::vector<double> temps;
    me::DeviceBuffer table;
    me::DeviceBuffer pair_counts;
    unsigned long long round = 0;
  } ladder;
  struct Population {
    me::DeviceBuffer fam, fam_out;
    me::DeviceBuffer x, energy;
    me::DeviceBuffer anc;
    me::DeviceBuffer scratch;
    me::DeviceBuffer records;
    unsigned long long stages = 0, capacity = 0;
    std::vector<double> temps;
  } population;
  struct Samples {
    me::DeviceBuffer data;
    long long capacity = 0, rows = 0;
    me::DeviceBuffer obs;
    int n_obs = 0;
    int obs_index[ME_MAX_RECORDED_OBSERVABLES] = {};
  } samples;
  std::string err;

  ~me_engine() {
    (void)hipSetDevice(device);
    if (comm && rccl) (void)rccl->comm_destroy(comm);
  }
};

namespace me {

int fail(me_engine *e, int code, const std::string &msg);

#define ME_HIP(e, call)                                                                                      \
  do {                                                                                                       \
    hipError_t err__ = (call);                                                                               \
    if (err__ != hipSuccess)                                                                                 \
      return me::fail((e), ME_ERR_HIP, std::string(#call) + ": " + hipGetErrorString(err__));                \
  } while (0)

int check_status(me_engine *e);

hipError_t upload(DeviceBuffer &dst, const double *src, size_t count, int dtype);

int refuse_stale_total(me_engine *e, const char *subject);

inline long long padded_chains(long long n) { return (n + 63) / 64 * 64; }

}

#pragma GCC visibility pop
```

metropolisengine_amd/csrc/me_generic.hip:

```cpp
#include "me_internal.h"
#include "me_launch.h"

namespace me {
namespace {

template <typename R>
__global__ void __launch_bounds__(kBlockThreads) k_broadcast_rows(R *dst, const R *row_values, int rows, long long n) {
  const long long stride = (long long)gridDim.x * kBlockThreads;
  for (long long c = (long long)blockIdx.x * kBlockThreads + threadIdx.x; c < n; c += stride)
    for (int r = 0; r < rows; ++r) dst[(long long)r * n + c] = row_values[r];
}

template <typename R>
__global__ void __launch_bounds__(kBlockThreads) k_broadcast_tiled(R *dst, const R *entry_values, int entries, long long n_padded) {
  const long long total = n_padded * entries, stride = (long long)gridDim.x * kBlockThreads;
  for (long long i = (long long)blockIdx.x * kBlockThreads + threadIdx.x; i < total; i += stride)
    dst[i] = entry_values[(i >> 6) % entries];
}

__device__ __forceinline__ void pair_of(int p, int &i, int &j) {
  i = (int)((sqrtf(8.0f * (float)p + 1.0f) - 1.0f) * 0.5f);
  while (i * (i + 1) / 2 > p) --i;
  while ((i + 1) * (i + 2) / 2 <= p) ++i;
  j = p - i * (i + 1) / 2;
}

constexpr int kMaxEntries = 12;

template <typename R, int TILE>
__global__ void __launch_bounds__(kBlockThreads) k_pool_reduce(const R *x, long long n, int nr, int nc, int entry_base, int tiled, double *partials) {
  extern __shared__ __attribute__((aligned(16))) unsigned char smem_raw[];
  R *tile = reinterpret_cast<R *>(smem_raw);
  constexpr int kTilePitch = TILE + 1;
  const int d = nr + 2 * nc;
  const int n_aug = d + nr + nc;
  const int n_pair = d * (d + 1) / 2;
  const int n_entries = 1 + n_aug + n_pair;
  const int tid = threadIdx.x;
  auto at = [&](int r, long long c) -> long long { return tiled ? ((c >> 6) * (long long)d + r) * 64 + (c & 63) : (long long)r * n + c; };

  int row_i[kMaxEntries], row_j[kMaxEntries];
  bool active[kMaxEntries];
  double acc[kMaxEntries];
#pragma unroll
  for (int k = 0; k < kMaxEntries; ++k) {
    const int e = entry_base + tid + k * kBlockThreads;
    acc[k] = 0.0;
    row_i[k] = row_j[k] = -1;
    active[k] = e < n_entries;
    if (!active[k] || e == 0) continue;
    if (e <= n_aug) {
      row_i[k] = e - 1;
    } else {
      pair_of(e - 1 - n_aug, row_i[k], row_j[k]);
// ... 143 lines not shown
constexpr int kSumThreads = 1024;
__global__ void __launch_bounds__(kSumThreads) k_sum_slots(const unsigned long long *slots, long long n_slots,
                                                           unsigned long long *total) {
  __shared__ unsigned long long part[kSumThreads / 64];
  unsigned long long s = 0;
  long long i = threadIdx.x;
  for (; i + 7 * kSumThreads < n_slots; i += 8 * kSumThreads) {
    unsigned long long v[8];
#pragma unroll
    for (int u = 0; u < 8; ++u) v[u] = slots[i + u * kSumThreads];
#pragma unroll
    for (int u = 0; u < 8; ++u) s += v[u];
  }
  for (; i < n_slots; i += kSumThreads) s += slots[i];
#pragma unroll
  for (int w = 32; w > 0; w >>= 1) s += __shfl_xor(s, w, 64);
  if ((threadIdx.x & 63) == 0) part[threadIdx.x >> 6] = s;
  __syncthreads();
  if (threadIdx.x == 0) {
    unsigned long long t = 0;
#pragma unroll
    for (int w = 0; w < kSumThreads / 64; ++w) t += part[w];
    total[0] = t;
  }
}

template <typename R>
__global__ void __launch_bounds__(kBlockThreads) k_trace(const R *x, const R *energy, const R *width, long long n, int d,
                                                         int n_terms, int width_rows, long long n_traced, long long stride,
                                                         int tiled, double *out) {
  const long long t = (long long)blockIdx.x * kBlockThreads + threadIdx.x;
  if (t >= n_traced) return;
  const long long c = t * stride;
  for (int k = 0; k < d; ++k)
    out[(long long)k * n_traced + t] = (double)x[tiled ? ((c >> 6) * (long long)d + k) * 64 + (c & 63) : (long long)k * n + c];
  for (int k = 0; k < n_terms; ++k) out[(long long)(d + k) * n_traced + t] = (double)energy[(long long)k * n + c];
  for (int r = 0; r < width_rows; ++r)
    out[(long long)(d + n_terms + r) * n_traced + t] = (double)width[(long long)r * n + c];
}

hipError_t launch_trace(const void *x, const void *energy, const void *width, long long n, int d, int n_terms,
                        int width_rows, int dtype, long long n_traced, long long stride, double *out, hipStream_t stream,
                        bool tiled_state) {
  const dim3 grid((unsigned)((n_traced + kBlockThreads - 1) / kBlockThreads)), block(kBlockThreads);
  if (dtype == ME_F32)
    hipLaunchKernelGGL(k_trace<float>, grid, block, 0, stream, (const float *)x, (const float *)energy, (const float *)width,
                       n, d, n_terms, width_rows, n_traced, stride, tiled_state ? 1 : 0, out);
  else
    hipLaunchKernelGGL(k_trace<double>, grid, block, 0, stream, (const double *)x, (const double *)energy,
                       (const double *)width, n, d, n_terms, width_rows, n_traced, stride, tiled_state ? 1 : 0, out);
  return hipGetLastError();
}

hipError_t launch_sum_slots(const unsigned long long *slots, long long n_slots, unsigned long long *total,
                            hipStream_t stream) {
  hipLaunchKernelGGL(k_sum_slots, dim3(1), dim3(kSumThreads), 0, stream, slots, n_slots, total);
  return hipGetLastError();
}

constexpr size_t kPoolLdsLimit = 160 * 1024;
int pool_tile_chains(int nr, int nc, int dtype) {
  const int n_aug = nr + 2 * nc + nr + nc;
  const size_t elem = dtype == ME_F32 ? sizeof(float) : sizeof(double);
  for (int tile : {64, 32, 16})
    if ((size_t)n_aug * (size_t)(tile + 1) * elem <= kPoolLdsLimit) return tile;
  return 0;
}

bool pool_reduce_supported(int nr, int nc, int dtype) { return pool_tile_chains(nr, nc, dtype) != 0; }

int pool_reduce_blocks(long long n, int nr, int nc) {
  const int d = nr + 2 * nc;
  const long long n_entries = 1 + d + nr + nc + (long long)d * (d + 1) / 2;
  long long cap = (32ll << 20) / (8 * n_entries);
  if (cap > 1024) cap = 1024;
  if (cap < 64) cap = 64;
  if (d + nr + nc <= 32) cap = 256;
  const long long tiles = (n + 63) / 64;
  return (int)(tiles < cap ? (tiles < 1 ? 1 : tiles) : cap);
}

namespace {
template <typename R, int TILE>
hipError_t launch_pool_stage1(const void *x, long long n, int nr, int nc, int n_entries, int blocks, double *partials, hipStream_t stream, bool tiled) {
  const size_t lds = (size_t)(nr + 2 * nc + nr + nc) * (size_t)(TILE + 1) * sizeof(R);
  if (lds > 64 * 1024)
    if (hipError_t rc = raise_lds_limit<k_pool_reduce<R, TILE>>(kPoolLdsLimit); rc != hipSuccess) return rc;
  for (int base = 0; base < n_entries; base += kMaxEntries * kBlockThreads)
    hipLaunchKernelGGL((k_pool_reduce<R, TILE>), dim3((unsigned)blocks), dim3(kBlockThreads), lds, stream, (const R *)x, n, nr, nc, base,
                       tiled ? 1 : 0, partials);
  return hipGetLastError();
}
template <typename R>
hipError_t launch_pool_stage1_tile(int tile, const void *x, long long n, int nr, int nc, int n_entries, int blocks, double *partials, hipStream_t stream, bool tiled) {
  switch (tile) {
    case 64: return launch_pool_stage1<R, 64>(x, n, nr, nc, n_entries, blocks, partials, stream, tiled);
    case 32: return launch_pool_stage1<R, 32>(x, n, nr, nc, n_entries, blocks, partials, stream, tiled);
    case 16: return launch_pool_stage1<R, 16>(x, n, nr, nc, n_entries, blocks, partials, stream, tiled);
    default: return hipErrorInvalidValue;
  }
}
}

hipError_t launch_pool_reduce(const void *x, long long n, int nr, int nc, int dtype, const unsigned long long *slots,
                              long long n_slots, double proposed, double *partials, double *out_device,
                              hipStream_t stream,
// ... 19 lines not shown
```

metropolisengine_amd/csrc/me_internal.h:

```cpp
#pragma once

#include <hip/hip_runtime.h>
#include <stdint.h>

#include "../../include/metropolis_engine.h"

namespace me {

enum CovKind { CK_IDENTITY = 0, CK_SHARED = 1, CK_PER_CHAIN = 2, CK_PER_CHAIN_NT = 3 };

enum StepGroup { GROUP_ALL = 0, GROUP_REAL = 1, GROUP_COMPLEX = 2 };

enum StatusBits : uint32_t {
  ST_NONFINITE_ENERGY = 1u,
  ST_BAD_PIVOT = 2u,
  ST_BAD_WIDTH = 4u
};

long long cache_budget_bytes();
void set_cache_budget_bytes(long long bytes);

constexpr int kBlockThreads = 256;
#ifndef ME_STEP_THREADS
#define ME_STEP_THREADS 64
#endif
constexpr int kStepThreads = ME_STEP_THREADS;
constexpr int kFusedStepThreads = 256;
constexpr int kFusedSweepsThreshold = 4;

struct StepLaunch {
  int n_real, n_complex;
  void *x, *energy, *width;
  const void *factor;
  const void *factor_full;
  const void *factor_image;
  const void *energy_image;
  const void *coef_device;
  const double *coef_host;
  int n_coef;
  const void *inj_normals;
  const void *inj_uniforms;
  unsigned long long *accept_slots;
  unsigned int *status;
  long long n;
  unsigned long long chain_offset, step_index, seed;
  int n_sweeps, energy_kind, cov_kind, reject_kind, grid_blocks;
  int group;
  int split_widths;
  int stale_total;
  const void *cov;
  double reject_bound, temp, ratio, target_acceptance, damping;
  const void *ladder;
  int tiles_per_rung;
};

struct MeasureLaunch {
  int n_real, n_complex;
  void *x, *width, *mean, *cov, *obs_mean, *factor;
  unsigned int *status;
  long long n;
  unsigned long long measure_count;
  int update_cov;
  int split_widths;
  int write_factor;
  int grid_blocks;
};

struct EnergyLaunch {
  int n_real, n_complex;
  int total_row;
  void *x, *energy;
  const void *coef_device;
  const double *coef_host;
  int n_coef;
  unsigned int *status;
  long long n;
  int energy_kind, grid_blocks;
};

constexpr int kMaxRegisterDof = 96;

struct KernelSet {
  const char *user_name;
  int dtype, n_real, n_complex;
  bool per_chain_cov;
  bool tracks_cov;
  bool (*has_energy)(int energy_kind);
  int (*energy_terms)(int energy_kind);
  hipError_t (*step)(const StepLaunch &, hipStream_t);
  hipError_t (*magphase)(const StepLaunch &, hipStream_t);
  hipError_t (*measure)(const MeasureLaunch &, hipStream_t);
  hipError_t (*init_energy)(const EnergyLaunch &, hipStream_t);
  size_t matrix_image_bytes;
  hipError_t (*prepare_matrix)(const void *matrix, void *image, hipStream_t);
  hipError_t (*pool_stage1)(const void *x, long long n, double *partials, int n_rows, hipStream_t);
  bool has_user_reject;
  bool streams_packed;
  hipError_t (*cycle)(const StepLaunch &, const MeasureLaunch &, hipStream_t);
  bool tiled_state;
};

void register_kernel_set(const KernelSet *set);
const KernelSet *find_kernel_set(int dtype, int n_real, int n_complex, int energy_kind, const char *user_name);
bool has_dims(int dtype, int n_real, int n_complex);

hipError_t launch_broadcast_rows(void *dst, const void *row_values, int rows, long long n, int dtype,
                                 hipStream_t stream);
hipError_t launch_broadcast_tiled(void *dst, const void *entry_values, int entries, long long n, int dtype,
                                  hipStream_t stream);
hipError_t launch_pool_reduce(const void *x, long long n, int n_real, int n_complex, int dtype,
                              const unsigned long long *slots, long long n_slots, double proposed, double *partials,
                              double *out_device, hipStream_t stream,
                              hipError_t (*stage1)(const void *, long long, double *, int, hipStream_t) = nullptr,
                              bool tiled_state = false);
int pool_reduce_blocks(long long n, int n_real, int n_complex);
bool pool_reduce_supported(int n_real, int n_complex, int dtype);
int pool_tile_chains(int n_real, int n_complex, int dtype);
hipError_t launch_trace(const void *x, const void *energy, const void *width, long long n, int d, int n_terms,
                        int width_rows, int dtype, long long n_traced, long long stride, double *out, hipStream_t stream,
                        bool tiled_state = false);
hipError_t launch_sum_slots(const unsigned long long *slots, long long n_slots, unsigned long long *total,
                            hipStream_t stream);

inline int grid_for(long long n, int requested, int threads = kStepThreads) {
  long long blocks = (n + threads - 1) / threads;
  if (requested > 0 && blocks > requested) blocks = requested;
  if (blocks < 1) blocks = 1;
  return (int)blocks;
}

__host__ __device__ inline int packed_real(int nr) { return nr * (nr + 1) / 2; }
__host__ __device__ inline int packed_total(int nr, int nc) { return nr * (nr + 1) / 2 + nc * nc; }
__host__ __device__ inline int n_observables(int nr, int nc) { return 2 * nr + nc; }
__host__ __device__ inline long long moments_size(int nr, int nc) {
  const int d = nr + 2 * nc;
  return 1 + d + (long long)d * (d + 1) / 2 + n_observables(nr, nc) + 2;
}

}
```

metropolisengine_amd/csrc/me_kernels.hip:

```cpp
#include <type_traits>

#include "me_device.h"
#include "me_dense_mfma.h"
#include "me_dense_bf16x3.h"
#include "me_dense_f64.h"
#include "me_factor_tile.h"
#include "me_per_device.h"
#include "me_pool_gram.h"
#include "me_magphase.h"

#ifdef ME_USER_SOURCE
#include ME_USER_SOURCE
#endif

#ifndef ME_NR
#error "compile with -DME_NR=<n_real> -DME_NC=<n_complex>"
#endif
#ifndef ME_DENSE
#define ME_DENSE 0
#endif
#ifndef ME_PER_CHAIN
#define ME_PER_CHAIN 1
#endif
#ifndef ME_TRACK_COV
#define ME_TRACK_COV 1
#endif

namespace me {
namespace {

constexpr int NR = ME_NR;
constexpr int NC = ME_NC;
[[maybe_unused]] constexpr int D = NR + 2 * NC;
constexpr bool kLandau = (NR == 2 && NC == 1);
constexpr bool kCylinder = (NR >= 1 && NC >= 1);

#ifdef ME_USER_SOURCE
#ifdef ME_USER_N_TERMS
}
}
template <typename R>
__device__ __forceinline__ R me_user_energy(const R *x, const R *coef) {
  R s = me_user_energy_term<R>(0, x, coef);
#pragma unroll
  for (int t = 1; t < ME_USER_N_TERMS; ++t) s += me_user_energy_term<R>(t, x, coef);
  return s;
}
namespace me {
namespace {
#endif
template <typename R, int NR_, int NC_>
struct EnergyUser {
  static constexpr int D = NR_ + 2 * NC_;
  const R *coef;
  __device__ __forceinline__ R operator()(const R (&x)[D]) const { return me_user_energy<R>(x, coef); }
#ifdef ME_USER_N_TERMS
  static constexpr int kTerms = ME_USER_N_TERMS;
  static constexpr unsigned term_groups(int t) { return me_user_term_groups(t); }
  __device__ __forceinline__ R term(int t, const R (&x)[D]) const { return me_user_energy_term<R>(t, x, coef); }
#endif
#ifdef ME_USER_HAS_REJECT
  __device__ __forceinline__ bool reject(const R (&x)[D]) const { return me_user_reject<R>(x, coef); }
#endif
};
template <typename R>
using user_fn_t = R (*)(const R *, const R *);
template <typename R>
__device__ R me_user_energy_entry(const R *x, const R *coef) { return me_user_energy<R>(x, coef); }
__device__ user_fn_t<float> g_user_fn_f32 = &me_user_energy_entry<float>;
__device__ user_fn_t<double> g_user_fn_f64 = &me_user_energy_entry<double>;
template <typename R, int NR_, int NC_>
struct EnergyUserIndirect {
  static constexpr int D = NR_ + 2 * NC_;
  user_fn_t<R> fn;
  const R *coef;
  __device__ __forceinline__ R operator()(const R (&x)[D]) const { return fn(x, coef); }
#ifdef ME_USER_HAS_REJECT
  __device__ __forceinline__ bool reject(const R (&x)[D]) const { return me_user_reject<R>(x, coef); }
#endif
};
template <typename R>
user_fn_t<R> load_user_fn() {
  user_fn_t<R> fn = nullptr;
  if constexpr (std::is_same<R, float>::value) (void)hipMemcpyFromSymbol(&fn, HIP_SYMBOL(g_user_fn_f32), sizeof(fn));
  else (void)hipMemcpyFromSymbol(&fn, HIP_SYMBOL(g_user_fn_f64), sizeof(fn));
  return fn;
}
#endif

int energy_terms(int kind) {
#ifdef ME_USER_SOURCE
#ifdef ME_USER_N_TERMS
  if (kind == ME_ENERGY_USER) return ME_USER_N_TERMS;
#else
  if (kind == ME_ENERGY_USER) return 1;
#endif
  return kind == ME_ENERGY_USER_INDIRECT ? 1 : 0;
#endif
  switch (kind) {
    case ME_ENERGY_ISO_QUAD:
    case ME_ENERGY_DIAG_QUAD: return 1;
    case ME_ENERGY_DENSE_QUAD: return ME_DENSE != 0 ? 1 : 0;
    case ME_ENERGY_LANDAU_TOY: return kLandau ? 1 : 0;
    case ME_ENERGY_LANDAU_TERMS: return kLandau ? 2 : 0;
    case ME_ENERGY_CYLINDER: return kCylinder ? 1 : 0;
    default: return 0;
  }
}
bool has_energy(int kind) { return energy_terms(kind) > 0; }

template <typename R, class Energy, bool INJECT, int GROUP, bool LADDER>
hipError_t launch_step_cov(const StepLaunch &l, const StepArgs<R> &a, const Energy &en, dim3 grid, dim3 block,
                           hipStream_t stream) {
  switch (l.cov_kind) {
    case CK_IDENTITY: {
      constexpr long long state_bytes = (long long)sizeof(R) * (D + 2);
      if constexpr (!INJECT && GROUP == GROUP_ALL && !LADDER) {
        if (state_bytes * l.n > 2 * cache_budget_bytes()) {
          hipLaunchKernelGGL((k_step<R, NR, NC, Energy, CK_IDENTITY, INJECT, GROUP, true>), grid, block, 0, stream, a, en);
          break;
        }
      }
      hipLaunchKernelGGL((k_step<R, NR, NC, Energy, CK_IDENTITY, INJECT, GROUP, false, LADDER>), grid, block, 0, stream, a, en);
      break;
    }
    case CK_SHARED: hipLaunchKernelGGL((k_step<R, NR, NC, Energy, CK_SHARED, INJECT, GROUP, false, LADDER>), grid, block, 0, stream, a, en); break;
#if ME_PER_CHAIN == 2
    case CK_PER_CHAIN: {
      if constexpr (INJECT) return hipErrorInvalidValue;
      else hipLaunchKernelGGL((k_step<R, NR, NC, Energy, CK_PER_CHAIN_NT, INJECT, GROUP, false, LADDER>), grid, block, 0, stream, a, en);
      break;
    }
#elif ME_PER_CHAIN
    case CK_PER_CHAIN: {
      constexpr long long per_chain_bytes = (long long)sizeof(R) * (D + 2 + NR * (NR + 1) / 2 + NC * NC);
      if constexpr (!INJECT) {
        if (per_chain_bytes * l.n > cache_budget_bytes()) {
          hipLaunchKernelGGL((k_step<R, NR, NC, Energy, CK_PER_CHAIN_NT, INJECT, GROUP, false, LADDER>), grid, block, 0, stream, a, en);
          break;
        }
      }
      hipLaunchKernelGGL((k_step<R, NR, NC, Energy, CK_PER_CHAIN, INJECT, GROUP, false, LADDER>), grid, block, 0, stream, a, en);
      break;
    }
#endif
    default: return hipErrorInvalidValue;
  }
  return hipGetLastError();
}

template <typename R, class Energy, bool INJECT, bool LADDER = false>
hipError_t launch_step_group(const StepLaunch &l, const StepArgs<R> &a, const Energy &en, dim3 grid, dim3 block,
                             hipStream_t stream) {
  if (l.group == GROUP_ALL) return launch_step_cov<R, Energy, INJECT, GROUP_ALL, LADDER>(l, a, en, grid, block, stream);
  if constexpr (NR > 0 && NC > 0) {
    if (l.group == GROUP_REAL) return launch_step_cov<R, Energy, INJECT, GROUP_REAL, LADDER>(l, a, en, grid, block, stream);
    if (l.group == GROUP_COMPLEX) return launch_step_cov<R, Energy, INJECT, GROUP_COMPLEX, LADDER>(l, a, en, grid, block, stream);
  }
  return hipErrorInvalidValue;
}

template <typename R, class Energy>
hipError_t step_with(const StepLaunch &l, const Energy &en, hipStream_t stream) {
  const StepArgs<R> a = typed<R>(l);
  const bool per_chain = l.cov_kind == CK_PER_CHAIN;
  const int threads = (l.n_sweeps >= kFusedSweepsThreshold || (ME_PER_CHAIN == 2 && per_chain)) ? kFusedStepThreads : kStepThreads;
  const dim3 grid(grid_for(l.n, l.grid_blocks, threads)), block(threads);
  if (l.ladder) {
    if (l.inj_normals) {
// ... 244 lines not shown
#else
#define ME_SET_NAME nullptr
#endif
constexpr auto pool_stage1_f32() -> hipError_t (*)(const void *, long long, double *, int, hipStream_t) {
  if constexpr (NR == 64 && NC == 0) return launch_pool_gram64;
  else if constexpr (D + NR + NC <= 32) return launch_pool_gram32<NR, NC>;
  else return nullptr;
}
constexpr auto pool_stage1_f64() -> hipError_t (*)(const void *, long long, double *, int, hipStream_t) {
  if constexpr (NR == 64 && NC == 0) return launch_pool_gram64_f64;
  else if constexpr (D + NR + NC <= 32) return launch_pool_gram32_f64<NR, NC>;
  else return nullptr;
}
#if ME_DENSE && !defined(ME_USER_SOURCE)
hipError_t prepare_matrix_f32(const void *factor_full, void *image, hipStream_t stream) {
  if constexpr (NR == 64 && NC == 0) {
    hipLaunchKernelGGL(k_dense64_bf16_fragments<0>, dim3(1), dim3(256), 0, stream, (const float *)factor_full,
                       (unsigned int *)image);
    return hipGetLastError();
  }
  return hipSuccess;
}
[[maybe_unused]] constexpr size_t kMatrixImageBytes = (NR == 64 && NC == 0) ? sizeof(unsigned int) * kBf16FragWords : 0;
#define ME_PREPARE_MATRIX_F32 kMatrixImageBytes, (kMatrixImageBytes ? prepare_matrix_f32 : nullptr), pool_stage1_f32()
hipError_t prepare_matrix_f64(const void *matrix, void *image, hipStream_t stream) {
  if constexpr (NR == 64 && NC == 0) {
    hipLaunchKernelGGL(k_dense64_f64_fragments<0>, dim3(1), dim3(256), 0, stream, (const double *)matrix, (double *)image);
    return hipGetLastError();
  }
  return hipSuccess;
}
[[maybe_unused]] constexpr size_t kMatrixImageBytesF64 = (NR == 64 && NC == 0) ? sizeof(double) * kDense64F64ImageDoubles : 0;
#define ME_PREPARE_MATRIX_F64 kMatrixImageBytesF64, (kMatrixImageBytesF64 ? prepare_matrix_f64 : nullptr), pool_stage1_f64()
#else
#define ME_PREPARE_MATRIX_F32 0, nullptr, pool_stage1_f32()
#define ME_PREPARE_MATRIX_F64 0, nullptr, pool_stage1_f64()
#endif
#ifdef ME_USER_HAS_REJECT
constexpr bool kHasUserReject = true;
#else
constexpr bool kHasUserReject = false;
#endif
#ifndef ME_ONLY_DTYPE
#define ME_ONLY_DTYPE 0
#endif
#if ME_ONLY_DTYPE != 64
const KernelSet kSetF32 = {ME_SET_NAME, ME_F32, NR, NC, ME_PER_CHAIN != 0, (ME_PER_CHAIN != 0 || ME_TRACK_COV != 0), has_energy, energy_terms, step<float>,
                           (NC > 0 && ME_PER_CHAIN == 1) ? magphase<float> : nullptr, measure<float>, init_energy<float>,
                           ME_PREPARE_MATRIX_F32, kHasUserReject, ME_PER_CHAIN == 2, cycle<float>, D >= kTiledStateDof};
#endif
#if ME_ONLY_DTYPE != 32
const KernelSet kSetF64 = {ME_SET_NAME, ME_F64, NR, NC, ME_PER_CHAIN != 0, (ME_PER_CHAIN != 0 || ME_TRACK_COV != 0), has_energy, energy_terms, step<double>,
                           (NC > 0 && ME_PER_CHAIN == 1) ? magphase<double> : nullptr, measure<double>, init_energy<double>,
                           ME_PREPARE_MATRIX_F64, kHasUserReject, ME_PER_CHAIN == 2, cycle<double>, D >= kTiledStateDof};
#endif

struct Registrar {
  Registrar() {
#if ME_ONLY_DTYPE != 64
    register_kernel_set(&kSetF32);
#endif
#if ME_ONLY_DTYPE != 32
    register_kernel_set(&kSetF64);
#endif
  }
} registrar;

}
}
```

metropolisengine_amd/csrc/me_mbar_obs.hip:

```cpp
#include "me_mbar.h"

#pragma clang fp contract(off)

namespace me {
namespace mbar {
namespace {

constexpr int kObsTargets = 4;
constexpr int kObsCols = 4;

struct ObsSelection {
  int q[ME_MAX_RECORDED_OBSERVABLES];
};

template <typename R>
__global__ void __launch_bounds__(kThreads) k_observable_record(const R *__restrict__ x, const R *__restrict__ energy, long long n,
                                                                 int nr, int nc, int n_terms, int tiled, ObsSelection sel,
                                                                 int n_sel, double *dst) {
  const long long c = (long long)blockIdx.x * kThreads + threadIdx.x;
  if (c >= n) return;
  const int d = nr + 2 * nc, nobs = 2 * nr + nc;
  const long long x0 = tiled ? (c >> 6) * (long long)d * 64 + (c & 63) : c;
  const long long xs = tiled ? 64 : n;
  for (int j = 0; j < n_sel; ++j) {
// ... 234 lines not shown
}

int reweight_observables_common(const Source &src, const double *f, const double *temps, int n, double *mean, double *var, double *cov,
                                double *neff) {
  const int rc = check_f_and_targets(src.e, f, src.n_rungs, temps, n, 1);
  if (rc) return rc;
  Problem p;
  return mbar_check_common(src.e, p, reweight_observables(p, src, f, temps, n, mean, var, cov, neff));
}

int catalogue_size(const me_engine *e) { return e->d + e->nobs + e->n_terms; }

}

hipError_t log_denominator_enqueue(Problem &p, const MbarSamples &sm, DeviceBuffer &d) {
  const long long n_padded = tiles_of(sm.n_samples) * kTile;
  ME_MBAR_HIP(d.resize((size_t)n_padded * sizeof(double)));
  hipLaunchKernelGGL(k_mbar_log_denominator, dim3(blocks_of(sm.n_samples)), dim3(kThreads), 0, p.stream, sm.energies, sm.n_samples,
                     n_padded, p.n_rungs, p.w.table.get<const double>(), d.get<double>());
  return hipGetLastError();
}

hipError_t reweight_observables_enqueue(Problem &p, const MbarSamples &sm, const ObsColumns &oc, const double *inv_temps, int n_temps,
                                        ObsScratch &scratch, double *out) {
  hipStream_t stream = p.stream;
  const int n_blocks = blocks_of(sm.n_samples), nq_all = oc.n_columns;
  const long long n_tiles = tiles_of(sm.n_samples);
  const size_t cells = (size_t)n_temps * nq_all;
  ME_MBAR_HIP(log_denominator_enqueue(p, sm, scratch.d));
  ME_MBAR_HIP(scratch.partials.resize((size_t)n_blocks * kObsTargets * sizeof(TargetState)));
  double *o_mean = out, *o_var = o_mean + cells, *o_cov = o_var + cells, *o_neff = o_cov + cells;
  for (int t0 = 0; t0 < n_temps; t0 += kObsTargets) {
    const int nt = std::min(kObsTargets, n_temps - t0);
    for (int q0 = 0; q0 < nq_all; q0 += kObsCols) {
      const int nq = std::min(kObsCols, nq_all - q0);
      const size_t cell = (size_t)t0 * nq_all + q0;
      hipLaunchKernelGGL(k_mbar_reweight_obs, dim3(n_blocks), dim3(kThreads), 0, stream, sm.energies, scratch.d.get<const double>(),
                         oc.data + (size_t)q0 * oc.column_stride, sm.n_samples, oc.n_chains, oc.record_stride, oc.column_stride, nq,
                         inv_temps + t0, nt, n_tiles, scratch.partials.get<TargetState>());
      hipLaunchKernelGGL(k_mbar_reweight_obs_finish, dim3(nt), dim3(kThreads), 0, stream, scratch.partials.get<const TargetState>(),
                         n_blocks, nq, nq_all, p.n_used, q0 == 0 ? 1 : 0, o_mean + cell, o_var + cell, o_cov + cell, o_neff + t0);
    }
  }
  return hipGetLastError();
}

hipError_t observable_record_enqueue(me_engine *e, long long row) {
  me_engine::Samples &s = e->samples;
  ObsSelection sel;
  for (int j = 0; j < ME_MAX_RECORDED_OBSERVABLES; ++j) sel.q[j] = j < s.n_obs ? s.obs_index[j] : 0;
  double *dst = s.obs.get<double>() + (size_t)row * (size_t)s.n_obs * (size_t)e->n;
  const dim3 grid((unsigned)((e->n + kThreads - 1) / kThreads));
  if (e->dtype == ME_F32)
    hipLaunchKernelGGL(k_observable_record<float>, grid, dim3(kThreads), 0, e->stream, e->x.get<const float>(), e->energy.get<const float>(),
                       e->n, e->nr, e->nc, e->n_terms, e->x_tiled ? 1 : 0, sel, s.n_obs, dst);
  else
    hipLaunchKernelGGL(k_observable_record<double>, grid, dim3(kThreads), 0, e->stream, e->x.get<const double>(),
                       e->energy.get<const double>(), e->n, e->nr, e->nc, e->n_terms, e->x_tiled ? 1 : 0, sel, s.n_obs, dst);
  return hipGetLastError();
}

}
}

using namespace me;
using namespace me::mbar;

extern "C" {

int me_observable_samples_enable(me_engine *e, const int32_t *indices, int32_t n_observables) {
  if (!e) return ME_ERR_INVALID;
  const int rc = refuse_stale_total(e, "observable samples are");
  if (rc != ME_OK) return rc;
  if (n_observables < 0 || n_observables > ME_MAX_RECORDED_OBSERVABLES)
    return fail(e, ME_ERR_INVALID, "n_observables must lie in [0, " + std::to_string(ME_MAX_RECORDED_OBSERVABLES) + "]");
  me_engine::Samples &s = e->samples;
  ME_HIP(e, hipSetDevice(e->device));
  if (n_observables == 0) {
    ME_HIP(e, hipStreamSynchronize(e->stream));
    s.obs.reset();
    s.n_obs = 0;
    return ME_OK;
  }
  if (!s.data) return fail(e, ME_ERR_STATE, "observable samples need the energy store: call me_energy_samples_enable first");
  if (!indices) return fail(e, ME_ERR_INVALID, "indices missing");
  for (int j = 0; j < n_observables; ++j)
    if (indices[j] < 0 || indices[j] >= catalogue_size(e))
      return fail(e, ME_ERR_INVALID, "observable index " + std::to_string(indices[j]) + " outside the catalogue of " +
                                         std::to_string(catalogue_size(e)) + " quantities");
  ME_HIP(e, hipStreamSynchronize(e->stream));
  s.obs.reset();
  s.n_obs = 0;
  s.rows = 0;
  const size_t bytes = (size_t)s.capacity * (size_t)n_observables * (size_t)e->n * sizeof(double);
  ME_HIP(e, s.obs.resize(bytes));
  if (bytes) {
    ME_HIP(e, hipMemsetAsync(s.obs.get(), 0, bytes, e->stream));
    ME_HIP(e, hipStreamSynchronize(e->stream));
  }
  s.n_obs = n_observables;
  for (int j = 0; j < n_observables; ++j) s.obs_index[j] = indices[j];
  return ME_OK;
}

int me_observable_samples_info(me_engine *e, int32_t *n_observables, int32_t *indices) {
  if (!e) return ME_ERR_INVALID;
  if (n_observables) *n_observables = e->samples.n_obs;
  if (indices)
    for (int j = 0; j < e->samples.n_obs; ++j) indices[j] = e->samples.obs_index[j];
  return ME_OK;
// ... 53 lines not shown
```

metropolisengine_amd/csrc/me_population.hip:

```cpp
#include <algorithm>
#include <cmath>
#include <vector>

#include "me_device.h"
#include "me_engine.h"

namespace me {
namespace {

constexpr int kPopThreads = 256;
constexpr int kPopWaves = kPopThreads / 64;
constexpr int kPopItems = 8;
constexpr int kPopChunk = kPopThreads * kPopItems;
constexpr int kFinalThreads = 256;
constexpr long long kSerialSlots = 8;

struct PopParams {
  double M, W, u;
  long long hi;
  long long n_finite;
};

template <typename R>
__device__ __forceinline__ double chain_log_weight(const Field<R> &fe, long long c, long long n, int n_terms, double neg_dbeta,
// ... 238 lines not shown
}

template <class F>
__device__ __forceinline__ void copy_rows(const F &src, const F &dst, unsigned int src_off, unsigned int dst_off, int rows) {
  constexpr int B = 8;
  for (int r0 = 0; r0 < rows; r0 += B) {
    decltype(src.load(0, 0u)) v[B];
#pragma unroll
    for (int k = 0; k < B; ++k)
      if (r0 + k < rows) v[k] = src.load(r0 + k, src_off);
#pragma unroll
    for (int k = 0; k < B; ++k)
      if (r0 + k < rows) dst.store(r0 + k, dst_off, v[k]);
  }
}

template <typename R>
__global__ void __launch_bounds__(kPopThreads) k_pop_gather(const R *x, const R *energy, const long long *fam, R *x_out,
                                                           R *energy_out, long long *fam_out, long long n, int d, int n_terms,
                                                           int tiled, const unsigned int *ancestors, const PopParams *params) {
  const long long j = (long long)blockIdx.x * kPopThreads + threadIdx.x;
  if (j >= n) return;
  const long long hi = params->hi;
  const long long a = (long long)ancestors[j < hi ? j : hi - 1];
  const unsigned int a_off = (unsigned int)a * (unsigned int)sizeof(R), j_off = (unsigned int)j * (unsigned int)sizeof(R);
  if (tiled) copy_rows(TiledField<R>(x, n, d), TiledField<R>(x_out, n, d), tiled_offset<R>(a, d), tiled_offset<R>(j, d), d);
  else copy_rows(Field<R>(x, n, d), Field<R>(x_out, n, d), a_off, j_off, d);
  copy_rows(Field<R>(energy, n, n_terms), Field<R>(energy_out, n, n_terms), a_off, j_off, n_terms);
  fam_out[j] = fam[a];
}

__global__ void __launch_bounds__(kPopThreads) k_pop_init_families(long long *fam, long long n, unsigned long long chain_offset) {
  const long long j = (long long)blockIdx.x * kPopThreads + threadIdx.x;
  if (j < n) fam[j] = (long long)(chain_offset + (unsigned long long)j);
}

template <typename R>
hipError_t launch(me_engine *e, double neg_dbeta) {
  me_engine::Population &pop = e->population;
  const long long n = e->n;
  hipStream_t stream = e->stream;
  const int n_blocks = (int)((n + kPopChunk - 1) / kPopChunk);
  const unsigned slot_blocks = (unsigned)((n + kPopThreads - 1) / kPopThreads);
  double *partials = pop.scratch.get<double>(), *factors = partials + 4 * (size_t)n_blocks, *offsets = factors + n_blocks;
  PopParams *params = (PopParams *)(offsets + n_blocks + 1);
  double *record = pop.records.get<double>() + 3 * (size_t)pop.stages;
  hipLaunchKernelGGL(k_pop_weights<R>, dim3(n_blocks), dim3(kPopThreads), 0, stream, e->energy.get<const R>(), n, e->n_terms,
                     neg_dbeta, partials);
  hipLaunchKernelGGL(k_pop_finalize, dim3(1), dim3(kFinalThreads), 0, stream, (const double *)partials, n_blocks, n,
                     e->chain_offset, pop.stages, (uint32_t)e->seed, (uint32_t)(e->seed >> 32), factors, offsets, params, record);
  hipLaunchKernelGGL(k_pop_scan_ancestors<R>, dim3(n_blocks), dim3(kPopThreads), 0, stream, e->energy.get<const R>(), n,
                     e->n_terms, neg_dbeta, (const double *)partials, (const double *)factors, (const double *)offsets,
                     (const PopParams *)params, pop.anc.get<unsigned int>());
  hipLaunchKernelGGL(k_pop_gather<R>, dim3(slot_blocks), dim3(kPopThreads), 0, stream, e->x.get<const R>(), e->energy.get<const R>(),
                     pop.fam.get<const long long>(), pop.x.get<R>(), pop.energy.get<R>(), pop.fam_out.get<long long>(), n, e->d,
                     e->n_terms, e->x_tiled ? 1 : 0, pop.anc.get<const unsigned int>(), (const PopParams *)params);
  return hipGetLastError();
}

size_t population_scratch_doubles(long long n) {
  const long long n_blocks = (n + kPopChunk - 1) / kPopChunk;
  return (size_t)(4 * n_blocks + n_blocks + n_blocks + 1) + (sizeof(PopParams) + sizeof(double) - 1) / sizeof(double);
}

int ensure_families(me_engine *e) {
  me_engine::Population &pop = e->population;
  if (pop.fam) return ME_OK;
  ME_HIP(e, pop.fam.resize((size_t)e->n * sizeof(long long)));
  hipLaunchKernelGGL(k_pop_init_families, dim3((unsigned)((e->n + kPopThreads - 1) / kPopThreads)), dim3(kPopThreads), 0, e->stream,
                     pop.fam.get<long long>(), e->n, e->chain_offset);
  ME_HIP(e, hipGetLastError());
  return ME_OK;
}
int ensure_population_scratch(me_engine *e) {
  me_engine::Population &pop = e->population;
  const size_t energy_bytes = (size_t)e->n * (size_t)e->n_terms * e->esize;
  if (pop.energy.bytes() < energy_bytes) {
    if (pop.energy) ME_HIP(e, hipStreamSynchronize(e->stream));
    ME_HIP(e, pop.energy.reserve(energy_bytes));
  }
  if (!pop.x) {
    ME_HIP(e, pop.x.resize(e->x.bytes()));
    ME_HIP(e, hipMemcpyAsync(pop.x.get(), e->x.get(), pop.x.bytes(), hipMemcpyDeviceToDevice, e->stream));
  }
  ME_HIP(e, pop.fam_out.resize((size_t)e->n * sizeof(long long)));
  ME_HIP(e, pop.anc.resize((size_t)e->n * sizeof(unsigned int)));
  ME_HIP(e, pop.scratch.resize(population_scratch_doubles(e->n) * sizeof(double)));
  return ME_OK;
}
int ensure_records(me_engine *e, unsigned long long stages) {
  me_engine::Population &pop = e->population;
  if (stages <= pop.capacity) return ME_OK;
  unsigned long long cap = std::max<unsigned long long>(256, pop.capacity);
  while (cap < stages) cap *= 2;
  DeviceBuffer grown;
  ME_HIP(e, grown.resize((size_t)cap * 3 * sizeof(double)));
  if (pop.records) {
    ME_HIP(e, hipMemcpyAsync(grown.get(), pop.records.get(), (size_t)pop.stages * 3 * sizeof(double), hipMemcpyDeviceToDevice, e->stream));
    ME_HIP(e, hipStreamSynchronize(e->stream));
  }
  pop.records = std::move(grown);
  pop.capacity = cap;
  return ME_OK;
}
int check_family_range(me_engine *e, int64_t chain_begin, int64_t n) {
  if (chain_begin < 0 || n < 0 || chain_begin + n > e->n) return fail(e, ME_ERR_INVALID, "family range outside the engine's chains");
  return ME_OK;
}

}
}

using namespace me;

extern "C" {

int me_set_temperature(me_engine *e, double temp) {
  if (!e) return ME_ERR_INVALID;
  if (!(std::isfinite(temp) && temp >= 0)) return fail(e, ME_ERR_INVALID, "temp must be finite and >= 0");
  if (e->ladder.n_rungs) return fail(e, ME_ERR_STATE, "this engine has a temperature ladder: its rungs carry the temperatures");
  e->temp = temp;
  return ME_OK;
}

int me_population_resample(me_engine *e, double new_temp) {
  if (!e) return ME_ERR_INVALID;
  if (!(std::isfinite(new_temp) && new_temp > 0)) return fail(e, ME_ERR_INVALID, "the new temperature must be finite and > 0");
  int rc = refuse_stale_total(e, "population annealing is");
  if (rc != ME_OK) return rc;
  if (e->ladder.n_rungs) return fail(e, ME_ERR_STATE, "population annealing needs the scalar temp: this engine has a temperature ladder");
  if (!(e->temp > 0)) return fail(e, ME_ERR_STATE, "population annealing cannot reweight from temp = 0: set a temperature first");
  ME_HIP(e, hipSetDevice(e->device));
  if ((rc = ensure_families(e)) || (rc = ensure_population_scratch(e)) || (rc = ensure_records(e, e->population.stages + 1))) return rc;
  me_engine::Population &pop = e->population;
  const double neg_dbeta = -(1.0 / new_temp - 1.0 / e->temp);
  ME_HIP(e, e->dtype == ME_F32 ? launch<float>(e, neg_dbeta) : launch<double>(e, neg_dbeta));
  ME_HIP(e, hipMemcpyAsync(e->x.get(), pop.x.get(), pop.x.bytes(), hipMemcpyDeviceToDevice, e->stream));
  ME_HIP(e, hipMemcpyAsync(e->energy.get(), pop.energy.get(), (size_t)e->n * (size_t)e->n_terms * e->esize, hipMemcpyDeviceToDevice, e->stream));
  ME_HIP(e, hipMemcpyAsync(pop.fam.get(), pop.fam_out.get(), (size_t)e->n * sizeof(long long), hipMemcpyDeviceToDevice, e->stream));
  e->temp = new_temp;
  e->population.temps.push_back(new_temp);
  e->population.stages += 1;
  return ME_OK;
}

int me_population_stats(me_engine *e, uint64_t *stages, double *stage_temps, double *log_weight, double *neff_fraction,
                        int64_t *n_finite, int64_t capacity) {
  if (!e) return ME_ERR_INVALID;
  if (stages) *stages = e->population.stages;
  if (!stage_temps && !log_weight && !neff_fraction && !n_finite) return ME_OK;
  if (capacity < 0 || (unsigned long long)capacity < e->population.stages)
    return fail(e, ME_ERR_INVALID, "the arrays must hold one entry per stage");
  if (e->population.stages == 0) return ME_OK;
  ME_HIP(e, hipSetDevice(e->device));
  std::vector<double> rec(3 * (size_t)e->population.stages);
  ME_HIP(e, hipMemcpyAsync(rec.data(), e->population.records.get(), rec.size() * sizeof(double), hipMemcpyDeviceToHost, e->stream));
  ME_HIP(e, hipStreamSynchronize(e->stream));
  for (size_t k = 0; k < e->population.stages; ++k) {
    if (stage_temps) stage_temps[k] = e->population.temps[k];
    if (log_weight) log_weight[k] = rec[3 * k];
    if (neff_fraction) neff_fraction[k] = rec[3 * k + 1];
    if (n_finite) n_finite[k] = (int64_t)rec[3 * k + 2];
  }
  return ME_OK;
}

int me_set_population_stats(me_engine *e, uint64_t stages, const double *stage_temps, const double *log_weight,
                            const double *neff_fraction, const int64_t *n_finite) {
  if (!e) return ME_ERR_INVALID;
  if (stages > 0 && (!stage_temps || !log_weight || !neff_fraction || !n_finite))
    return fail(e, ME_ERR_INVALID, "stage_temps / log_weight / neff_fraction / n_finite missing");
  std::vector<double> rec(3 * (size_t)stages);
  for (uint64_t k = 0; k < stages; ++k) {
    if (!(std::isfinite(stage_temps[k]) && stage_temps[k] > 0)) return fail(e, ME_ERR_INVALID, "stage temperatures must be finite and > 0");
    if (n_finite[k] < 0 || n_finite[k] > e->n) return fail(e, ME_ERR_INVALID, "n_finite must lie in [0, n_chains]");
    rec[3 * k] = log_weight[k];
    rec[3 * k + 1] = neff_fraction[k];
    rec[3 * k + 2] = (double)n_finite[k];
  }
  ME_HIP(e, hipSetDevice(e->device));
  int rc = ensure_records(e, std::max<uint64_t>(stages, 1));
  if (rc) return rc;
  if (stages > 0) {
    ME_HIP(e, hipMemcpyAsync(e->population.records.get(), rec.data(), rec.size() * sizeof(double), hipMemcpyHostToDevice, e->stream));
    ME_HIP(e, hipStreamSynchronize(e->stream));
  }
  e->population.temps.assign(stage_temps, stage_temps + stages);
  e->population.stages = stages;
  return ME_OK;
}
// ... 28 lines not shown
```

metropolisengine_amd/csrc/me_replica.hip:

```cpp
#include <algorithm>
#include <cmath>
#include <string>
#include <vector>

#include "me_device.h"
#include "me_engine.h"

namespace me {
namespace {

constexpr int kSwapThreads = 256;
constexpr int kSwapBlocks = 2048;

template <typename R>
struct SwapArgs {
  R *x, *energy;
  const R *ladder;
  unsigned long long *pair_counts;
  long long n, rung_chains;
  unsigned long long chain_offset, round;
  uint32_t seed_lo, seed_hi;
  int d, n_terms, first_rung, tiled;
};

// ... 107 lines not shown
}
}
}

using namespace me;

extern "C" {

int me_set_temperature_ladder(me_engine *e, const double *temps, int32_t n_rungs) {
  if (!e) return ME_ERR_INVALID;
  if (n_rungs < 0 || (n_rungs > 0 && !temps)) return fail(e, ME_ERR_INVALID, "n_rungs must be >= 0 and temps given");
  ME_HIP(e, hipSetDevice(e->device));
  if (n_rungs == 0) return free_ladder(e);
  int rc = check_ladder_capable(e);
  if (rc != ME_OK) return rc;
  for (int k = 0; k < n_rungs; ++k) {
    if (!(std::isfinite(temps[k]) && temps[k] > 0))
      return fail(e, ME_ERR_INVALID, "ladder temperatures must be finite and > 0");
    if (k > 0 && !(temps[k] > temps[k - 1]))
      return fail(e, ME_ERR_INVALID, "ladder temperatures must be strictly increasing");
  }
  if (e->n % (64ll * n_rungs) != 0)
    return fail(e, ME_ERR_INVALID, "n_chains must be a multiple of 64 * n_rungs: every rung is a run of whole 64-chain tiles");
  std::vector<double> table(2 * (size_t)n_rungs);
  for (int k = 0; k < n_rungs; ++k) {
    table[2 * k] = 1.0 / temps[k];
    table[2 * k + 1] = 1.4426950408889634 / temps[k];
  }
  if ((rc = free_ladder(e)) != ME_OK) return rc;
  ME_HIP(e, upload(e->ladder.table, table.data(), table.size(), e->dtype));
  ME_HIP(e, e->ladder.pair_counts.resize(2 * (size_t)std::max(n_rungs - 1, 1) * sizeof(unsigned long long)));
  ME_HIP(e, hipMemset(e->ladder.pair_counts.get(), 0, e->ladder.pair_counts.bytes()));
  e->ladder.temps.assign(temps, temps + n_rungs);
  e->ladder.n_rungs = n_rungs;
  return ME_OK;
}

int me_temperature_ladder(me_engine *e, double *temps, int32_t capacity, int32_t *n_rungs) {
  if (!e || !n_rungs) return ME_ERR_INVALID;
  *n_rungs = e->ladder.n_rungs;
  if (e->ladder.n_rungs == 0 || !temps) return ME_OK;
  if (capacity < e->ladder.n_rungs) return fail(e, ME_ERR_INVALID, "temps must hold n_rungs doubles");
  std::copy(e->ladder.temps.begin(), e->ladder.temps.end(), temps);
  return ME_OK;
}

int me_replica_exchange(me_engine *e, int32_t n_rounds) {
  if (!e) return ME_ERR_INVALID;
  if (n_rounds < 0) return fail(e, ME_ERR_INVALID, "n_rounds must be >= 0");
  if (e->ladder.n_rungs == 0) return fail(e, ME_ERR_STATE, "no temperature ladder: call me_set_temperature_ladder first");
  ME_HIP(e, hipSetDevice(e->device));
  const auto swap = e->dtype == ME_F32 ? launch<float> : launch<double>;
  for (int i = 0; i < n_rounds; ++i) {
    ME_HIP(e, swap(e->x.get(), e->energy.get(), e->n, e->d, e->n_terms, e->x_tiled, e->ladder.table.get(), e->ladder.n_rungs, e->ladder.round,
                   e->chain_offset, e->seed, e->ladder.pair_counts.get<unsigned long long>(), e->stream));
    e->ladder.round += 1;
  }
  return ME_OK;
}

int me_replica_stats(me_engine *e, uint64_t *round, uint64_t *attempted, uint64_t *accepted, int32_t n_pairs) {
  if (!e) return ME_ERR_INVALID;
  if (e->ladder.n_rungs == 0) return fail(e, ME_ERR_STATE, "no temperature ladder");
  if (n_pairs != e->ladder.n_rungs - 1) return fail(e, ME_ERR_INVALID, "n_pairs must be n_rungs - 1");
  if (round) *round = e->ladder.round;
  if (n_pairs == 0) return ME_OK;
  ME_HIP(e, hipSetDevice(e->device));
  std::vector<unsigned long long> counts(2 * (size_t)n_pairs);
  ME_HIP(e, hipMemcpyAsync(counts.data(), e->ladder.pair_counts.get(), counts.size() * sizeof(unsigned long long), hipMemcpyDeviceToHost,
                           e->stream));
  ME_HIP(e, hipStreamSynchronize(e->stream));
  for (int k = 0; k < n_pairs; ++k) {
    if (attempted) attempted[k] = counts[2 * k];
    if (accepted) accepted[k] = counts[2 * k + 1];
  }
  return ME_OK;
}

int me_set_replica_stats(me_engine *e, uint64_t round, const uint64_t *attempted, const uint64_t *accepted, int32_t n_pairs) {
  if (!e) return ME_ERR_INVALID;
  if (e->ladder.n_rungs == 0) return fail(e, ME_ERR_STATE, "no temperature ladder");
  if (n_pairs != e->ladder.n_rungs - 1) return fail(e, ME_ERR_INVALID, "n_pairs must be n_rungs - 1");
  if (n_pairs > 0 && (!attempted || !accepted)) return fail(e, ME_ERR_INVALID, "attempted / accepted missing");
  std::vector<unsigned long long> counts(2 * (size_t)n_pairs);
  for (int k = 0; k < n_pairs; ++k) {
    if (accepted[k] > attempted[k]) return fail(e, ME_ERR_INVALID, "accepted swaps exceed attempted ones");
    counts[2 * k] = attempted[k];
    counts[2 * k + 1] = accepted[k];
  }
  ME_HIP(e, hipSetDevice(e->device));
  if (n_pairs > 0) {
    ME_HIP(e, hipMemcpyAsync(e->ladder.pair_counts.get(), counts.data(), counts.size() * sizeof(unsigned long long), hipMemcpyHostToDevice,
                             e->stream));
    ME_HIP(e, hipStreamSynchronize(e->stream));
  }
  e->ladder.round = round;
  return ME_OK;
}

}
```

metropolisengine_amd/engine.py:

```python
import ctypes

import numpy as np

from . import _capi
from .energy import EnergySpec, RejectSpec

_DTYPES = {"f32": _capi.ME_F32, "float32": _capi.ME_F32, "f64": _capi.ME_F64, "float64": _capi.ME_F64}
_COV_MODES = {"reference": _capi.COV_REFERENCE, "fixed": _capi.COV_FIXED, "pooled": _capi.COV_POOLED}


_as_double_ptr = _capi.double_ptr


def _initial_state(initial_real_params, initial_complex_params):
    try:
        r = np.asarray([] if initial_real_params is None else initial_real_params, dtype=np.float64).reshape(-1)
        c = np.asarray([] if initial_complex_params is None else initial_complex_params, dtype=np.complex128).reshape(-1)
    except (TypeError, ValueError):
        return None
    return np.concatenate([r, c.real, c.imag])


def unpack_real_block(packed, nr):
    n = packed.shape[0]
# ... 202 lines not shown
            pass

    def _check(self, status):
        _capi.check(status, self._handle)

    def step_all(self, n_sweeps=1):
        self._check(self._lib.me_step(self._handle, int(n_sweeps)))
        if self.n_chains == 1:
            accepted, _ = self.accept_stats()
            took = accepted > self._last_accepted
            self._last_accepted = accepted
            return took if n_sweeps == 1 else None
        return None

    def step_injected(self, normals, uniforms, kind=_capi.STEP_ALL):
        normals = np.ascontiguousarray(normals, dtype=np.float64)
        uniforms = np.ascontiguousarray(uniforms, dtype=np.float64)
        nc = self.num_complex_params
        magphase = kind == _capi.STEP_COMPLEX_MAGNITUDE_PHASE
        nz = nc if magphase else self.num_real_params + 2 * nc
        want_u = normals.shape[:2] + ((nc + 2,) if magphase else ())
        if normals.ndim != 3 or normals.shape[1:] != (self.n_chains, nz) or uniforms.shape != want_u:
            raise ValueError("injected streams have the wrong shape for this step kind")
        self._check(self._lib.me_step_injected(self._handle, int(kind), normals.shape[0], _as_double_ptr(normals),
                                               _as_double_ptr(uniforms)))

    def _step_kind(self, kind, n_sweeps):
        before = self.accept_stats()[0] if self.n_chains == 1 else 0
        self._check(self._lib.me_step_kind(self._handle, int(kind), int(n_sweeps)))
        if self.n_chains == 1 and n_sweeps == 1 and kind != _capi.STEP_COMPLEX_MAGNITUDE_PHASE:
            accepted = self.accept_stats()[0]
            self._last_accepted = accepted
            return accepted > before
        return None

    def step_real_group(self, n_sweeps=1):
        return self._step_kind(_capi.STEP_REAL_GROUP, n_sweeps)

    def step_complex_group(self, n_sweeps=1):
        if self.complex_sample_method == "magnitude-phase":
            return self._step_kind(_capi.STEP_COMPLEX_MAGNITUDE_PHASE, n_sweeps)
        return self._step_kind(_capi.STEP_COMPLEX_GROUP, n_sweeps)

    def measure(self):
        self._check(self._lib.me_measure(self._handle))

    def cycle(self, n_sweeps=1):
        self._check(self._lib.me_cycle(self._handle, int(n_sweeps)))

    def fused_cycles(self):
        count = ctypes.c_uint64()
        self._check(self._lib.me_cycle_stats(self._handle, ctypes.byref(count)))
        return count.value

    measure_real_system = measure
    measure_complex_system = measure

    def set_reject_condition(self, reject_fct):
        if reject_fct is not None and not isinstance(reject_fct, RejectSpec):
            from .pyenergy import PythonEnergy, PythonReject
            if not callable(reject_fct):
                raise TypeError("reject_condition must be a RejectSpec, a callable or None")
            if not isinstance(self._energy_spec, PythonEnergy):
                raise TypeError("a Python reject_condition needs a Python energy (both are traced into one device plugin); "
                                "with a built-in energy use a RejectSpec such as AbsReal0AtLeast")
            self._bind_energy(PythonEnergy(self._energy_spec.energy, reject=reject_fct))
            reject_fct = PythonReject()
        kind = reject_fct.kind if reject_fct is not None else _capi.REJECT_NONE
        bound = reject_fct.bound if reject_fct is not None else 0.0
        self._check(self._lib.me_set_reject_condition(self._handle, int(kind), float(bound)))
        self._reject_spec = reject_fct

    def _bind_energy(self, spec):
        nr, nc = self.num_real_params, self.num_complex_params
        name = None
        if hasattr(spec, "ensure_loaded"):
            spec.ensure_loaded(nr, nc)
            name = spec.name.encode()
        coeffs = np.ascontiguousarray(spec.coefficients(nr, nc), dtype=np.float64)
        self._check(self._lib.me_set_energy(self._handle, int(spec.kind), _as_double_ptr(coeffs), int(coeffs.size), name))
        self._energy_spec = spec
        self._user_name = name
        self.energy_term_names = list(spec.term_names)

    def set_energy_function(self, energy_function):
        if not isinstance(energy_function, EnergySpec):
            if not (callable(energy_function) or isinstance(energy_function, dict)):
                raise TypeError("energy_function must be an EnergySpec, a callable or a dictionary of term callables")
            from .pyenergy import PythonEnergy
            keep = getattr(self._energy_spec, "reject", None) if isinstance(self._reject_spec, RejectSpec) and \
                self._reject_spec.kind == _capi.REJECT_USER else None
            energy_function = PythonEnergy(energy_function, reject=keep)
        self._bind_energy(energy_function)

    def initialize_energy_dict(self):
        self._check(self._lib.me_recompute_energy(self._handle))

    def set_initial_sampling_width(self, sampling_width):
        self.group_sampling_width = sampling_width

    def _get(self, field, chain_begin=0, n_chains=None):
        n = self.n_chains - chain_begin if n_chains is None else n_chains
        comps = ctypes.c_int32()
        self._check(self._lib.me_field_components(self._handle, field, ctypes.byref(comps)))
        out = np.empty((n, comps.value), dtype=np.float64)
        self._check(self._lib.me_get(self._handle, field, chain_begin, n, _as_double_ptr(out)))
# ... 771 lines not shown
```

Measured before the change: 19.21 billion.

## Add per-chain line state layout with adaptive retiling for step kernels

Adds an alternative state layout in which each chain's 16 float64 parameters sit in one contiguous 128-byte line. A new step kernel loads whole tiles with 128-bit buffer loads, transposes them through a swizzled LDS slab, and writes back only the lines whose chain changed. A policy switches the state into line form after a streak of eligible step launches and flips it back to row form whenever a row consumer (measure, trace, pooled moments, replica exchange, field access) needs it. The aim is cheaper global memory traffic per sweep for short-sweep launches, at the cost of retile kernels on every format switch and more bookkeeping throughout the API.

```diff
diff --git a/include/metropolis_engine.h b/include/metropolis_engine.h
--- a/include/metropolis_engine.h
+++ b/include/metropolis_engine.h
@@ -137,6 +137,11 @@
 int me_pooled_moments_allreduce_begin(me_engine *engine);
 int me_set_shared_factor(me_engine *engine, const double *packed_factor, int64_t n_doubles);
 int me_set_cache_budget(int64_t bytes);
+#define ME_STATE_FORMAT_NEVER 0
+#define ME_STATE_FORMAT_ALWAYS 1
+#define ME_STATE_FORMAT_AUTO 2
+int me_set_state_format(me_engine *engine, int32_t mode);
+int me_state_format(me_engine *engine, int32_t *lines_active, uint64_t *line_launches, uint64_t *retiles);
 int me_get_shared_factor(me_engine *engine, double *packed_factor, int64_t n_doubles, int32_t *is_set);
 
 int me_trace_enable(me_engine *engine, int64_t n_traced, int64_t stride);
diff --git a/metropolisengine_amd/_capi.py b/metropolisengine_amd/_capi.py
--- a/metropolisengine_amd/_capi.py
+++ b/metropolisengine_amd/_capi.py
@@ -91,6 +91,9 @@
     "me_get_shared_factor": (ctypes.c_int, [_H, _dp, ctypes.c_int64, ctypes.POINTER(ctypes.c_int32)]),
     "me_set_accept_stats": (ctypes.c_int, [_H, ctypes.c_uint64, ctypes.c_uint64]),
     "me_set_cache_budget": (ctypes.c_int, [ctypes.c_int64]),
+    "me_set_state_format": (ctypes.c_int, [_H, ctypes.c_int32]),
+    "me_state_format": (ctypes.c_int, [_H, ctypes.POINTER(ctypes.c_int32), ctypes.POINTER(ctypes.c_uint64),
+                                       ctypes.POINTER(ctypes.c_uint64)]),
     "me_trace_enable": (ctypes.c_int, [_H, ctypes.c_int64, ctypes.c_int64]),
     "me_trace_shape": (ctypes.c_int, [_H, ctypes.POINTER(ctypes.c_int64), ctypes.POINTER(ctypes.c_int64),
                                       ctypes.POINTER(ctypes.c_int64)]),
diff --git a/metropolisengine_amd/csrc/me_api.hip b/metropolisengine_amd/csrc/me_api.hip
--- a/metropolisengine_amd/csrc/me_api.hip
+++ b/metropolisengine_amd/csrc/me_api.hip
@@ -156,10 +156,35 @@
   return fail(e, ME_ERR_NUMERIC, msg);
 }
 int check_status(me_engine *e) {
+  if (e->retile_error != hipSuccess)
+    return fail(e, ME_ERR_HIP, std::string("the state could not be flipped between row and line form: ") + hipGetErrorString(e->retile_error));
   unsigned long long *scratch = e->host_scratch.get<unsigned long long>();
   ME_HIP(e, hipMemcpyAsync(&scratch[0], e->status.get(), sizeof(unsigned int), hipMemcpyDeviceToHost, e->stream));
   ME_HIP(e, hipStreamSynchronize(e->stream));
   return report_status(e, (unsigned int)scratch[0]);
+}
+
+namespace {
+void flip_state(me_engine *e, lines::Policy::Flip flip) {
+  if (flip == lines::Policy::kStay) return;
+  const hipError_t err = launch_retile(e->x_store.get(), e->n, e->d, e->dtype, flip == lines::Policy::kToLines, e->stream);
+  if (err != hipSuccess && e->retile_error == hipSuccess) e->retile_error = err;
+}
+bool lines_eligible(const me_engine *e, const StepLaunch &l) {
+  return e->ks->lines_step && e->x_tiled && l.cov_kind == CK_IDENTITY && l.group == GROUP_ALL && !l.inj_normals && !l.ladder &&
+         (long long)e->esize * (e->d + 2) * e->n <= 2 * cache_budget_bytes();
+}
+}
+
+void *state_rows(me_engine *e) {
+  flip_state(e, e->lines.row_consumer());
+  return e->x_store.get();
+}
+
+void state_for_step(me_engine *e, StepLaunch &l) {
+  flip_state(e, e->lines.step(lines_eligible(e, l), l.n_sweeps < kFusedSweepsThreshold));
+  l.x = e->x_store.get();
+  l.x_lines = e->lines.in_lines ? 1 : 0;
 }
 
 }
@@ -220,7 +245,7 @@
 
 int field_info(me_engine *e, int field, void **ptr, int *comps) {
   switch (field) {
-    case ME_FIELD_PARAMS: *ptr = e->x.get(); *comps = e->d; return ME_OK;
+    case ME_FIELD_PARAMS: *ptr = e->x_store.get(); *comps = e->d; return ME_OK;
     case ME_FIELD_ENERGY: *ptr = e->energy.get(); *comps = e->n_terms; return ME_OK;
     case ME_FIELD_WIDTH: *ptr = e->width.get(); *comps = e->width_rows; return ME_OK;
     case ME_FIELD_MEAN: *ptr = e->mean.get(); *comps = e->d; return ME_OK;
@@ -256,10 +281,10 @@
   return ME_OK;
 }
 
-void fill_step_launch(me_engine *e, StepLaunch &l, int n_sweeps) {
+void fill_step_launch(me_engine *e, StepLaunch &l, int n_sweeps, int group = GROUP_ALL, const void *inj_normals = nullptr,
+                      const void *inj_uniforms = nullptr, bool rows_only = false) {
   l.n_real = e->nr;
   l.n_complex = e->nc;
-  l.x = e->x.get();
   l.energy = e->energy.get();
   l.width = e->width.get();
   l.factor = e->cov_kind == CK_PER_CHAIN ? e->factor.get() : e->shared_factor.get();
@@ -269,9 +294,9 @@
   l.coef_device = e->coef_dev.get();
   l.coef_host = e->coef.data();
   l.n_coef = (int)e->coef.size();
-  l.inj_normals = nullptr;
-  l.inj_uniforms = nullptr;
-  l.group = GROUP_ALL;
+  l.inj_normals = inj_normals;
+  l.inj_uniforms = inj_uniforms;
+  l.group = group;
   l.split_widths = (e->width_rows == 3 && !e->widths_synced) ? 1 : 0;
   l.stale_total = e->stale_total ? 1 : 0;
   l.cov = e->cov.get();
@@ -293,6 +318,12 @@
   l.damping = std::max((double)e->measure_count / (double)e->m, 200.0);
   l.ladder = e->ladder.n_rungs ? e->ladder.table.get() : nullptr;
   l.tiles_per_rung = e->ladder.n_rungs ? (int)(e->n / (64ll * e->ladder.n_rungs)) : 0;
+  if (rows_only) {
+    l.x = state_rows(e);
+    l.x_lines = 0;
+  } else {
+    state_for_step(e, l);
+  }
 }
 
 int check_reject_kind(me_engine *e, int reject_kind, int energy_kind, int n_real) {
@@ -470,7 +501,7 @@
   ME_HIP(e, hipSetDevice(e->device));
   ME_HIP(e, e->stream.create());
   const size_t n = (size_t)e->n, tiles = (size_t)padded_chains(e->n), es = e->esize;
-  ME_HIP(e, e->x.resize((e->x_tiled ? tiles : n) * e->d * es));
+  ME_HIP(e, e->x_store.resize((e->x_tiled ? tiles : n) * e->d * es));
   ME_HIP(e, e->energy.resize(n * (e->n_terms + (e->stale_total ? 1 : 0)) * es));
   ME_HIP(e, e->width.resize(n * e->width_rows * es));
   ME_HIP(e, e->mean.resize(n * e->d * es));
@@ -560,7 +591,7 @@
     return fail(e, ME_ERR_INVALID, "initial covariance matrix is not positive definite (metropolis_engine.py:270)");
   int rc = ME_OK;
   std::vector<double> width_row((size_t)e->width_rows, c->sampling_width);
-  if ((rc = broadcast(e, e->x, init, e->x_tiled)) || (rc = broadcast(e, e->mean, init)) || (rc = broadcast(e, e->obs_mean, obs)) ||
+  if ((rc = broadcast(e, e->x_store, init, e->x_tiled)) || (rc = broadcast(e, e->mean, init)) || (rc = broadcast(e, e->obs_mean, obs)) ||
       (rc = broadcast(e, e->width, width_row)) || (e->cov && (rc = broadcast(e, e->cov, c0, true))) ||
       (e->factor && (rc = broadcast(e, e->factor, f0, true))) || (rc = upload_shared_factor(e, f0.data())))
     return rc;
@@ -668,7 +699,7 @@
   l.n_real = e->nr;
   l.n_complex = e->nc;
   l.total_row = e->stale_total ? e->n_terms : -1;
-  l.x = e->x.get();
+  l.x = state_rows(e);
   l.energy = e->energy.get();
   l.coef_device = e->coef_dev.get();
   l.coef_host = e->coef.data();
@@ -722,17 +753,15 @@
   e->proposed += (unsigned long long)e->n * (unsigned long long)n_sweeps * (magphase ? 2ull : 1ull);
 }
 
-static int launch_step_kind(me_engine *e, int kind, int n_sweeps, const void *inj_normals, const void *inj_uniforms) {
+static int launch_step_kind(me_engine *e, int kind, int n_sweeps, const void *inj_normals, const void *inj_uniforms,
+                            bool rows_only = false) {
   int group;
   bool magphase;
   int rc = resolve_step_kind(e, kind, &group, &magphase);
   if (rc != ME_OK) return rc;
   if ((group != GROUP_ALL || magphase) && (rc = split_widths(e)) != ME_OK) return rc;
   StepLaunch l;
-  fill_step_launch(e, l, n_sweeps);
-  l.group = group;
-  l.inj_normals = inj_normals;
-  l.inj_uniforms = inj_uniforms;
+  fill_step_launch(e, l, n_sweeps, group, inj_normals, inj_uniforms, magphase || rows_only);
   hipError_t err = magphase ? e->ks->magphase(l, e->stream) : e->ks->step(l, e->stream);
   if (err == hipErrorNotSupported) return fail(e, ME_ERR_UNSUPPORTED, "this step kind is not compiled for this engine");
   ME_HIP(e, err);
@@ -778,7 +807,7 @@
 void fill_measure_launch(me_engine *e, MeasureLaunch &l, unsigned long long count) {
   l.n_real = e->nr;
   l.n_complex = e->nc;
-  l.x = e->x.get();
+  l.x = state_rows(e);
   l.width = e->width.get();
   l.mean = e->mean.get();
   l.cov = e->cov.get();
@@ -812,7 +841,7 @@
     }
     const int rows_valid = (e->width_rows == 3 && e->widths_synced) ? 1 : e->width_rows;
     double *row = e->trace.dev.get<double>() + e->trace.rows * cols * e->trace.chains;
-    ME_HIP(e, launch_trace(e->x.get(), e->energy.get(), e->width.get(), e->n, e->d, e->n_terms, rows_valid, e->dtype, e->trace.chains,
+    ME_HIP(e, launch_trace(state_rows(e), e->energy.get(), e->width.get(), e->n, e->d, e->n_terms, rows_valid, e->dtype, e->trace.chains,
                            e->trace.stride, row, e->stream, e->x_tiled));
     if (rows_valid != e->width_rows) {
       double *widths = row + (size_t)(e->d + e->n_terms) * e->trace.chains;
@@ -841,7 +870,7 @@
   ME_HIP(e, hipSetDevice(e->device));
   if (e->ks->cycle) {
     StepLaunch sl;
-    fill_step_launch(e, sl, n_sweeps);
+    fill_step_launch(e, sl, n_sweeps, GROUP_ALL, nullptr, nullptr, true);
     MeasureLaunch ml;
     fill_measure_launch(e, ml, e->measure_count + 1);
     ml.split_widths = 0;
@@ -854,7 +883,7 @@
     if (err != hipErrorNotSupported) ME_HIP(e, err);
     (void)hipGetLastError();
   }
-  const int rc = me_step(e, n_sweeps);
+  const int rc = launch_step_kind(e, ME_STEP_ALL, n_sweeps, nullptr, nullptr, true);
   return rc != ME_OK ? rc : me_measure(e);
 }
 
@@ -919,6 +948,7 @@
   int rc = field_info(e, field, &ptr, &comps);
   if (rc != ME_OK) return rc;
   if (n_chains == 0) return ME_OK;
+  if (field == ME_FIELD_PARAMS) ptr = state_rows(e);
   if (field == ME_FIELD_COV || field == ME_FIELD_FACTOR || (field == ME_FIELD_PARAMS && e->x_tiled))
     return copy_tiled(e, ptr, comps, chain_begin, n_chains, dst, nullptr);
   std::vector<unsigned char> tmp((size_t)comps * n_chains * e->esize);
@@ -945,6 +975,7 @@
   if (field == ME_FIELD_WIDTH && e->width_rows == 3 && (chain_begin != 0 || n_chains != e->n))
     return fail(e, ME_ERR_INVALID, "widths of a mixed engine must be set for all chains at once");
   if (n_chains == 0) return ME_OK;
+  if (field == ME_FIELD_PARAMS) ptr = state_rows(e);
   if (field == ME_FIELD_COV || field == ME_FIELD_FACTOR || (field == ME_FIELD_PARAMS && e->x_tiled)) {
     rc = copy_tiled(e, ptr, comps, chain_begin, n_chains, nullptr, src);
     if (rc != ME_OK) return rc;
@@ -1061,7 +1092,7 @@
 }
 int enqueue_pooled_moments(me_engine *e, double *device_out, int64_t n_doubles) {
   const int rc = check_pooled(e, n_doubles);
-  return rc != ME_OK ? rc : enqueue_pool_reduce(e, e->x.get(), e->n, e->n_slots, (double)e->proposed, device_out);
+  return rc != ME_OK ? rc : enqueue_pool_reduce(e, state_rows(e), e->n, e->n_slots, (double)e->proposed, device_out);
 }
 int fetch_pooled_moments(me_engine *e, double *host_out, int64_t n_doubles) {
   const size_t bytes = sizeof(double) * (size_t)n_doubles;
@@ -1092,7 +1123,7 @@
     return fail(e, ME_ERR_INVALID, "the chain range must be whole 64-chain tiles inside the engine");
   int rc = check_pooled(e, n_doubles);
   if (rc != ME_OK) return rc;
-  const unsigned char *x = e->x.get<unsigned char>();
+  const unsigned char *x = state_rows<unsigned char>(e);
   if (e->x_tiled) {
     x += (size_t)chain_begin * e->d * e->esize;
   } else {
@@ -1262,6 +1293,30 @@
   return ME_OK;
 }
 
+int me_set_state_format(me_engine *e, int32_t mode) {
+  if (!e) return ME_ERR_INVALID;
+  if (mode != ME_STATE_FORMAT_NEVER && mode != ME_STATE_FORMAT_ALWAYS && mode != ME_STATE_FORMAT_AUTO)
+    return fail(e, ME_ERR_INVALID, "unknown state format mode");
+  static_assert(ME_STATE_FORMAT_NEVER == lines::kNever && ME_STATE_FORMAT_ALWAYS == lines::kAlways && ME_STATE_FORMAT_AUTO == lines::kAuto,
+                "the public modes are the policy's");
+  ME_HIP(e, hipSetDevice(e->device));
+  const lines::Policy::Flip flip = e->lines.set_mode(mode);
+  if (flip == lines::Policy::kToRows) {
+    const hipError_t err = launch_retile(e->x_store.get(), e->n, e->d, e->dtype, false, e->stream);
+    if (err != hipSuccess && e->retile_error == hipSuccess) e->retile_error = err;
+    ME_HIP(e, err);
+  }
+  return ME_OK;
+}
+
+int me_state_format(me_engine *e, int32_t *lines_active, uint64_t *line_launches, uint64_t *retiles) {
+  if (!e) return ME_ERR_INVALID;
+  if (lines_active) *lines_active = e->lines.in_lines ? 1 : 0;
+  if (line_launches) *line_launches = e->lines.line_launches;
+  if (retiles) *retiles = e->lines.retiles;
+  return ME_OK;
+}
+
 int me_time_steps(me_engine *e, int32_t n_launches, int32_t n_sweeps, float *elapsed_ms) {
   if (!e || !elapsed_ms) return ME_ERR_INVALID;
   if (n_launches <= 0 || n_sweeps <= 0) return fail(e, ME_ERR_INVALID, "n_launches and n_sweeps must be positive");
diff --git a/metropolisengine_amd/csrc/me_device.h b/metropolisengine_amd/csrc/me_device.h
--- a/metropolisengine_amd/csrc/me_device.h
+++ b/metropolisengine_amd/csrc/me_device.h
@@ -8,6 +8,7 @@
 
 #include "me_internal.h"
 #include "me_math64.h"
+#include "me_state_lines.h"
 
 namespace me {
 
@@ -907,6 +908,108 @@
   publish_step(a, blockDim.x >> 6, wave_accepted, bad_energy, bad_width);
 }
 
+namespace lines {
+constexpr int kWaveLdsBytes = kTileBytes + kTileChains;
+}
+typedef unsigned int lines_u32x4 __attribute__((ext_vector_type(4)));
+typedef double lines_f64x2 __attribute__((ext_vector_type(2)));
+__device__ __forceinline__ void lines_handover() {
+  __builtin_amdgcn_fence(__ATOMIC_RELEASE, "wavefront");
+  __builtin_amdgcn_wave_barrier();
+  __builtin_amdgcn_fence(__ATOMIC_ACQUIRE, "wavefront");
+}
+
+template <typename R, int NR, int NC, class Energy>
+__global__ void ME_STEP_BOUNDS k_step_lines(StepArgs<R> a, Energy en) {
+  static_assert(NC == 0 && sizeof(R) == 8 && NR * sizeof(R) == lines::kLineBytes, "one 128-byte line per chain: 16 real float64 parameters");
+  constexpr int D = NR;
+  using N_ = Num<R>;
+  extern __shared__ __attribute__((aligned(16))) unsigned char lines_lds[];
+
+  stagger_priority();
+  N_::prepare();
+  energy_prepare(en, 0);
+  unsigned int wave_accepted = 0;
+  bool bad_energy = false, bad_width = false;
+  using Ledger = EnergyLedger<R, Energy, GROUP_ALL>;
+  const StateField<R, false> fe(a.energy, a.n, Ledger::T), fw(a.width, a.n, 1);
+  const int tiles = (int)((a.n + 63) >> 6);
+  const __amdgpu_buffer_rsrc_t fx = __builtin_amdgcn_make_buffer_rsrc(a.x, 0, (unsigned int)tiles * (unsigned int)lines::kTileBytes, 0x00020000);
+  const int lane = (int)(threadIdx.x & 63u);
+  const int wave = __builtin_amdgcn_readfirstlane((int)(threadIdx.x >> 6)), waves = (int)(blockDim.x >> 6);
+  lines_u32x4 *slab = reinterpret_cast<lines_u32x4 *>(lines_lds + wave * lines::kWaveLdsBytes);
+  unsigned char *order = reinterpret_cast<unsigned char *>(slab + lines::kTileChunks);
+  const unsigned int lane_chunk = (unsigned int)lane * lines::kChunkBytes;
+
+  for (int t = (int)blockIdx.x * waves + wave; t < tiles; t += (int)gridDim.x * waves) {
+    const unsigned int tile_off = (unsigned int)__builtin_amdgcn_readfirstlane(t * lines::kTileBytes);
+    int in_lane = lane;
+    asm volatile("" : "+v"(in_lane));
+    {
+      lines_u32x4 v[lines::kChunksPerLine];
+#pragma unroll
+      for (int k = 0; k < lines::kChunksPerLine; ++k)
+        v[k] = __builtin_amdgcn_raw_buffer_load_b128(fx, lane_chunk, tile_off + (unsigned int)k * 1024u, 0);
+#pragma unroll
+      for (int k = 0; k < lines::kChunksPerLine; ++k) slab[lines::slab_chunk_of_line_chunk(k * 64 + in_lane)] = v[k];
+    }
+    lines_handover();
+    const long long c = (long long)t * 64 + lane;
+    bool changed = false;
+    if (c < a.n) {
+      const unsigned int coff = (unsigned int)c * (unsigned int)sizeof(R);
+      R x[D];
+#pragma unroll
+      for (int p = 0; p < lines::kChunksPerLine; ++p) {
+        const lines_f64x2 q = __builtin_bit_cast(lines_f64x2, slab[lines::slab_chunk(in_lane, p)]);
+        x[2 * p] = q.x;
+        x[2 * p + 1] = q.y;
+      }
+      Ledger ledger;
+      R total_q5 = R(0);
+      ledger.load(fe, coff);
+      R w = fw.load(0, coff);
+      R w_r = w, w_c = w;
+      const unsigned long long gid = a.chain_offset + (unsigned long long)c;
+      auto fac = [&](int k) -> R { return a.factor[k]; };
+      run_sweeps<R, NR, NC, Energy, CK_IDENTITY, false, GROUP_ALL, false>(a, en, c, gid, false, x, ledger, total_q5, w, w_r, w_c, fac,
+                                                                          wave_accepted, bad_energy);
+      bad_width |= !(w > R(0));
+      ledger.store(fe, coff);
+      fw.store(0, coff, w);
+      int own = lane;
+      asm volatile("" : "+v"(own)::"memory");
+      lines_u32x4 now[lines::kChunksPerLine];
+#pragma unroll
+      for (int p = 0; p < lines::kChunksPerLine; ++p) {
+        now[p] = __builtin_bit_cast(lines_u32x4, lines_f64x2{x[2 * p], x[2 * p + 1]});
+        const lines_u32x4 was = slab[lines::slab_chunk(own, p)];
+        changed |= (now[p].x != was.x) | (now[p].y != was.y) | (now[p].z != was.z) | (now[p].w != was.w);
+      }
+      if (changed) {
+#pragma unroll
+        for (int p = 0; p < lines::kChunksPerLine; ++p) slab[lines::slab_chunk(own, p)] = now[p];
+      }
+    }
+    const unsigned long long moved = __ballot(changed);
+    const int n_moved = __popcll(moved);
+    if (changed) order[__builtin_amdgcn_mbcnt_hi((unsigned int)(moved >> 32), __builtin_amdgcn_mbcnt_lo((unsigned int)moved, 0u))] = (unsigned char)lane;
+    lines_handover();
+    int out_lane = lane;
+    asm volatile("" : "+v"(out_lane));
+    for (int j = 0; j * 8 < n_moved; ++j) {
+      const int slot = j * 8 + (out_lane >> 3);
+      if (slot < n_moved) {
+        const int chain = order[slot], pair = out_lane & 7;
+        __builtin_amdgcn_raw_buffer_store_b128(slab[lines::slab_chunk(chain, pair)], fx,
+                                               (unsigned int)(chain * lines::kChunksPerLine + pair) * lines::kChunkBytes, tile_off, 0);
+      }
+    }
+    lines_handover();
+  }
+  publish_step(a, (unsigned int)waves, wave_accepted, bad_energy, bad_width);
+}
+
 template <typename R, int NR, int NC, class Energy>
 __global__ void __launch_bounds__(kStepThreads) k_init_energy(const R *xs, R *energy, long long n, unsigned int *status,
                                                                 Energy en, int total_row) {
diff --git a/metropolisengine_amd/csrc/me_engine.h b/metropolisengine_amd/csrc/me_engine.h
--- a/metropolisengine_amd/csrc/me_engine.h
+++ b/metropolisengine_amd/csrc/me_engine.h
@@ -6,6 +6,7 @@
 
 #include "me_comm.h"
 #include "me_internal.h"
+#include "me_state_lines.h"
 
 #pragma GCC visibility push(hidden)
 
@@ -137,7 +138,9 @@
   std::vector<double> coef;
   unsigned long long step_index = 0, measure_count = 1;
   unsigned long long fused_cycles = 0;
-  me::DeviceBuffer x, energy, width, mean, cov, obs_mean;
+  me::DeviceBuffer x_store, energy, width, mean, cov, obs_mean;
+  me::lines::Policy lines;
+  hipError_t retile_error = hipSuccess;
   me::DeviceBuffer factor, shared_factor, shared_full, shared_image, energy_image, coef_dev, row_dev;
   me::DeviceBuffer accept_slots, accept_total;
   long long n_slots = 0;
@@ -214,6 +217,11 @@
 
 int refuse_stale_total(me_engine *e, const char *subject);
 
+void *state_rows(me_engine *e);
+template <typename T>
+T *state_rows(me_engine *e) { return static_cast<T *>(state_rows(e)); }
+void state_for_step(me_engine *e, StepLaunch &l);
+
 inline long long padded_chains(long long n) { return (n + 63) / 64 * 64; }
 
 }
diff --git a/metropolisengine_amd/csrc/me_generic.hip b/metropolisengine_amd/csrc/me_generic.hip
--- a/metropolisengine_amd/csrc/me_generic.hip
+++ b/metropolisengine_amd/csrc/me_generic.hip
@@ -1,5 +1,8 @@
+#include <algorithm>
+
 #include "me_internal.h"
 #include "me_launch.h"
+#include "me_state_lines.h"
 
 namespace me {
 namespace {
@@ -249,6 +252,65 @@
   return hipGetLastError();
 }
 
+namespace {
+template <typename R, int D, bool TO_LINES>
+__global__ void __launch_bounds__(64) k_retile(R *x, long long tiles) {
+  static_assert(D * sizeof(R) == lines::kLineBytes, "a chain's state is one 128-byte line");
+  constexpr int VPC = lines::kChunkBytes / (int)sizeof(R);
+  typedef R Chunk __attribute__((ext_vector_type(VPC)));
+  __shared__ __attribute__((aligned(16))) Chunk slab[lines::kTileChunks];
+  const int lane = threadIdx.x;
+  for (long long t = blockIdx.x; t < tiles; t += gridDim.x) {
+    R *rows = x + t * (long long)(D * 64);
+    Chunk *chunks = reinterpret_cast<Chunk *>(rows);
+    if constexpr (TO_LINES) {
+      R v[D];
+#pragma unroll
+      for (int d = 0; d < D; ++d) v[d] = rows[d * 64 + lane];
+#pragma unroll
+      for (int p = 0; p < lines::kChunksPerLine; ++p) {
+        Chunk ch;
+#pragma unroll
+        for (int i = 0; i < VPC; ++i) ch[i] = v[p * VPC + i];
+        slab[lines::slab_chunk(lane, p)] = ch;
+      }
+      __syncthreads();
+      Chunk q[lines::kChunksPerLine];
+#pragma unroll
+      for (int k = 0; k < lines::kChunksPerLine; ++k) q[k] = slab[lines::slab_chunk_of_line_chunk(k * 64 + lane)];
+#pragma unroll
+      for (int k = 0; k < lines::kChunksPerLine; ++k) chunks[k * 64 + lane] = q[k];
+    } else {
+      Chunk q[lines::kChunksPerLine];
+#pragma unroll
+      for (int k = 0; k < lines::kChunksPerLine; ++k) q[k] = chunks[k * 64 + lane];
+#pragma unroll
+      for (int k = 0; k < lines::kChunksPerLine; ++k) slab[lines::slab_chunk_of_line_chunk(k * 64 + lane)] = q[k];
+      __syncthreads();
+      R v[D];
+#pragma unroll
+      for (int p = 0; p < lines::kChunksPerLine; ++p) {
+        const Chunk ch = slab[lines::slab_chunk(lane, p)];
+#pragma unroll
+        for (int i = 0; i < VPC; ++i) v[p * VPC + i] = ch[i];
+      }
+#pragma unroll
+      for (int d = 0; d < D; ++d) rows[d * 64 + lane] = v[d];
+    }
+    __syncthreads();
+  }
+}
+}
+
+hipError_t launch_retile(void *x, long long n, int d, int dtype, bool to_lines, hipStream_t stream) {
+  if (dtype != ME_F64 || d * 8 != lines::kLineBytes || !x || n <= 0) return hipErrorInvalidValue;
+  const long long tiles = (n + 63) / 64;
+  const dim3 grid((unsigned)std::min<long long>(tiles, 1ll << 20)), block(64);
+  if (to_lines) hipLaunchKernelGGL((k_retile<double, 16, true>), grid, block, 0, stream, (double *)x, tiles);
+  else hipLaunchKernelGGL((k_retile<double, 16, false>), grid, block, 0, stream, (double *)x, tiles);
+  return hipGetLastError();
+}
+
 hipError_t launch_sum_slots(const unsigned long long *slots, long long n_slots, unsigned long long *total,
                             hipStream_t stream) {
   hipLaunchKernelGGL(k_sum_slots, dim3(1), dim3(kSumThreads), 0, stream, slots, n_slots, total);
diff --git a/metropolisengine_amd/csrc/me_internal.h b/metropolisengine_amd/csrc/me_internal.h
--- a/metropolisengine_amd/csrc/me_internal.h
+++ b/metropolisengine_amd/csrc/me_internal.h
@@ -52,6 +52,7 @@
   double reject_bound, temp, ratio, target_acceptance, damping;
   const void *ladder;
   int tiles_per_rung;
+  int x_lines;
 };
 
 struct MeasureLaunch {
@@ -98,6 +99,7 @@
   bool streams_packed;
   hipError_t (*cycle)(const StepLaunch &, const MeasureLaunch &, hipStream_t);
   bool tiled_state;
+  bool lines_step;
 };
 
 void register_kernel_set(const KernelSet *set);
@@ -119,6 +121,7 @@
 hipError_t launch_trace(const void *x, const void *energy, const void *width, long long n, int d, int n_terms,
                         int width_rows, int dtype, long long n_traced, long long stride, double *out, hipStream_t stream,
                         bool tiled_state = false);
+hipError_t launch_retile(void *x, long long n, int d, int dtype, bool to_lines, hipStream_t stream);
 hipError_t launch_sum_slots(const unsigned long long *slots, long long n_slots, unsigned long long *total,
                             hipStream_t stream);
 
diff --git a/metropolisengine_amd/csrc/me_kernels.hip b/metropolisengine_amd/csrc/me_kernels.hip
--- a/metropolisengine_amd/csrc/me_kernels.hip
+++ b/metropolisengine_amd/csrc/me_kernels.hip
@@ -34,6 +34,8 @@
 [[maybe_unused]] constexpr int D = NR + 2 * NC;
 constexpr bool kLandau = (NR == 2 && NC == 1);
 constexpr bool kCylinder = (NR >= 1 && NC >= 1);
+template <typename R>
+constexpr bool kLinesStep = NC == 0 && sizeof(R) == 8 && NR * sizeof(R) == lines::kLineBytes && D >= kTiledStateDof;
 
 #ifdef ME_USER_SOURCE
 #ifdef ME_USER_N_TERMS
@@ -115,6 +117,15 @@
   switch (l.cov_kind) {
     case CK_IDENTITY: {
       constexpr long long state_bytes = (long long)sizeof(R) * (D + 2);
+      if (l.x_lines) {
+        if constexpr (kLinesStep<R> && !INJECT && GROUP == GROUP_ALL && !LADDER) {
+          if (state_bytes * l.n > 2 * cache_budget_bytes()) return hipErrorInvalidValue;
+          hipLaunchKernelGGL((k_step_lines<R, NR, NC, Energy>), grid, block, (block.x >> 6) * lines::kWaveLdsBytes, stream, a, en);
+          break;
+        } else {
+          return hipErrorInvalidValue;
+        }
+      }
       if constexpr (!INJECT && GROUP == GROUP_ALL && !LADDER) {
         if (state_bytes * l.n > 2 * cache_budget_bytes()) {
           hipLaunchKernelGGL((k_step<R, NR, NC, Energy, CK_IDENTITY, INJECT, GROUP, true>), grid, block, 0, stream, a, en);
@@ -465,7 +476,8 @@
 #if ME_ONLY_DTYPE != 32
 const KernelSet kSetF64 = {ME_SET_NAME, ME_F64, NR, NC, ME_PER_CHAIN != 0, (ME_PER_CHAIN != 0 || ME_TRACK_COV != 0), has_energy, energy_terms, step<double>,
                            (NC > 0 && ME_PER_CHAIN == 1) ? magphase<double> : nullptr, measure<double>, init_energy<double>,
-                           ME_PREPARE_MATRIX_F64, kHasUserReject, ME_PER_CHAIN == 2, cycle<double>, D >= kTiledStateDof};
+                           ME_PREPARE_MATRIX_F64, kHasUserReject, ME_PER_CHAIN == 2, cycle<double>, D >= kTiledStateDof,
+                           kLinesStep<double>};
 #endif
 
 struct Registrar {
diff --git a/metropolisengine_amd/csrc/me_mbar_obs.hip b/metropolisengine_amd/csrc/me_mbar_obs.hip
--- a/metropolisengine_amd/csrc/me_mbar_obs.hip
+++ b/metropolisengine_amd/csrc/me_mbar_obs.hip
@@ -310,10 +310,10 @@
   double *dst = s.obs.get<double>() + (size_t)row * (size_t)s.n_obs * (size_t)e->n;
   const dim3 grid((unsigned)((e->n + kThreads - 1) / kThreads));
   if (e->dtype == ME_F32)
-    hipLaunchKernelGGL(k_observable_record<float>, grid, dim3(kThreads), 0, e->stream, e->x.get<const float>(), e->energy.get<const float>(),
+    hipLaunchKernelGGL(k_observable_record<float>, grid, dim3(kThreads), 0, e->stream, state_rows<const float>(e), e->energy.get<const float>(),
                        e->n, e->nr, e->nc, e->n_terms, e->x_tiled ? 1 : 0, sel, s.n_obs, dst);
   else
-    hipLaunchKernelGGL(k_observable_record<double>, grid, dim3(kThreads), 0, e->stream, e->x.get<const double>(),
+    hipLaunchKernelGGL(k_observable_record<double>, grid, dim3(kThreads), 0, e->stream, state_rows<const double>(e),
                        e->energy.get<const double>(), e->n, e->nr, e->nc, e->n_terms, e->x_tiled ? 1 : 0, sel, s.n_obs, dst);
   return hipGetLastError();
 }
diff --git a/metropolisengine_amd/csrc/me_population.hip b/metropolisengine_amd/csrc/me_population.hip
--- a/metropolisengine_amd/csrc/me_population.hip
+++ b/metropolisengine_amd/csrc/me_population.hip
@@ -314,7 +314,7 @@
   hipLaunchKernelGGL(k_pop_scan_ancestors<R>, dim3(n_blocks), dim3(kPopThreads), 0, stream, e->energy.get<const R>(), n,
                      e->n_terms, neg_dbeta, (const double *)partials, (const double *)factors, (const double *)offsets,
                      (const PopParams *)params, pop.anc.get<unsigned int>());
-  hipLaunchKernelGGL(k_pop_gather<R>, dim3(slot_blocks), dim3(kPopThreads), 0, stream, e->x.get<const R>(), e->energy.get<const R>(),
+  hipLaunchKernelGGL(k_pop_gather<R>, dim3(slot_blocks), dim3(kPopThreads), 0, stream, state_rows<const R>(e), e->energy.get<const R>(),
                      pop.fam.get<const long long>(), pop.x.get<R>(), pop.energy.get<R>(), pop.fam_out.get<long long>(), n, e->d,
                      e->n_terms, e->x_tiled ? 1 : 0, pop.anc.get<const unsigned int>(), (const PopParams *)params);
   return hipGetLastError();
@@ -342,8 +342,8 @@
     ME_HIP(e, pop.energy.reserve(energy_bytes));
   }
   if (!pop.x) {
-    ME_HIP(e, pop.x.resize(e->x.bytes()));
-    ME_HIP(e, hipMemcpyAsync(pop.x.get(), e->x.get(), pop.x.bytes(), hipMemcpyDeviceToDevice, e->stream));
+    ME_HIP(e, pop.x.resize(e->x_store.bytes()));
+    ME_HIP(e, hipMemcpyAsync(pop.x.get(), state_rows(e), pop.x.bytes(), hipMemcpyDeviceToDevice, e->stream));
   }
   ME_HIP(e, pop.fam_out.resize((size_t)e->n * sizeof(long long)));
   ME_HIP(e, pop.anc.resize((size_t)e->n * sizeof(unsigned int)));
@@ -397,7 +397,7 @@
   me_engine::Population &pop = e->population;
   const double neg_dbeta = -(1.0 / new_temp - 1.0 / e->temp);
   ME_HIP(e, e->dtype == ME_F32 ? launch<float>(e, neg_dbeta) : launch<double>(e, neg_dbeta));
-  ME_HIP(e, hipMemcpyAsync(e->x.get(), pop.x.get(), pop.x.bytes(), hipMemcpyDeviceToDevice, e->stream));
+  ME_HIP(e, hipMemcpyAsync(state_rows(e), pop.x.get(), pop.x.bytes(), hipMemcpyDeviceToDevice, e->stream));
   ME_HIP(e, hipMemcpyAsync(e->energy.get(), pop.energy.get(), (size_t)e->n * (size_t)e->n_terms * e->esize, hipMemcpyDeviceToDevice, e->stream));
   ME_HIP(e, hipMemcpyAsync(pop.fam.get(), pop.fam_out.get(), (size_t)e->n * sizeof(long long), hipMemcpyDeviceToDevice, e->stream));
   e->temp = new_temp;
diff --git a/metropolisengine_amd/csrc/me_replica.hip b/metropolisengine_amd/csrc/me_replica.hip
--- a/metropolisengine_amd/csrc/me_replica.hip
+++ b/metropolisengine_amd/csrc/me_replica.hip
@@ -183,7 +183,7 @@
   ME_HIP(e, hipSetDevice(e->device));
   const auto swap = e->dtype == ME_F32 ? launch<float> : launch<double>;
   for (int i = 0; i < n_rounds; ++i) {
-    ME_HIP(e, swap(e->x.get(), e->energy.get(), e->n, e->d, e->n_terms, e->x_tiled, e->ladder.table.get(), e->ladder.n_rungs, e->ladder.round,
+    ME_HIP(e, swap(state_rows(e), e->energy.get(), e->n, e->d, e->n_terms, e->x_tiled, e->ladder.table.get(), e->ladder.n_rungs, e->ladder.round,
                    e->chain_offset, e->seed, e->ladder.pair_counts.get<unsigned long long>(), e->stream));
     e->ladder.round += 1;
   }
diff --git a/metropolisengine_amd/csrc/me_state_lines.h b/metropolisengine_amd/csrc/me_state_lines.h
--- /dev/null
+++ b/metropolisengine_amd/csrc/me_state_lines.h
@@ -0,0 +1,83 @@
+#pragma once
+
+namespace me {
+namespace lines {
+
+constexpr int kLineBytes = 128;
+constexpr int kTileChains = 64;
+constexpr int kTileBytes = kLineBytes * kTileChains;
+constexpr int kChunkBytes = 16;
+constexpr int kChunksPerLine = kLineBytes / kChunkBytes;
+constexpr int kTileChunks = kTileBytes / kChunkBytes;
+constexpr int kTileValues = kTileBytes / 8;
+
+constexpr int kD = kLineBytes / 8;
+constexpr int row_element(int lane, int d) { return d * kTileChains + lane; }
+constexpr int line_element(int lane, int d) { return lane * kD + d; }
+constexpr int rows_to_lines(int row_el) { return line_element(row_el % kTileChains, row_el / kTileChains); }
+constexpr int lines_to_rows(int line_el) { return row_element(line_el / kD, line_el % kD); }
+
+constexpr int slab_chunk(int lane, int pair) { return lane * kChunksPerLine + (pair ^ ((lane >> 1) & 7)); }
+constexpr int slab_chunk_of_line_chunk(int chunk) { return slab_chunk(chunk / kChunksPerLine, chunk % kChunksPerLine); }
+
+static_assert(kD == 16 && kTileChunks == 512 && kTileValues == 1024, "a tile is 64 lines of 16 doubles");
+static_assert(rows_to_lines(row_element(5, 3)) == line_element(5, 3) && lines_to_rows(line_element(63, 15)) == row_element(63, 15),
+              "rows <-> lines");
+static_assert(lines_to_rows(rows_to_lines(777)) == 777 && rows_to_lines(lines_to_rows(1023)) == 1023, "inverse maps");
+static_assert(slab_chunk_of_line_chunk(slab_chunk_of_line_chunk(345)) == 345, "the slab placement is an involution");
+static_assert(slab_chunk(63, 7) < kTileChunks && slab_chunk(0, 0) == 0, "the slab is the tile's size");
+
+enum Mode { kNever = 0, kAlways = 1, kAuto = 2 };
+
+#ifndef ME_LINES_ENTER_AFTER
+#define ME_LINES_ENTER_AFTER 20
+#endif
+constexpr int kEnterAfter = ME_LINES_ENTER_AFTER;
+
+struct Policy {
+  enum Flip { kStay = 0, kToLines = 1, kToRows = 2 };
+  int mode = kAuto;
+  bool in_lines = false;
+  int streak = 0;
+  unsigned long long line_launches = 0;
+  unsigned long long retiles = 0;
+
+  Flip row_consumer() {
+    streak = 0;
+    return leave();
+  }
+  Flip step(bool eligible, bool profits = true) {
+    if (!eligible || mode == kNever) {
+      streak = 0;
+      return leave();
+    }
+    if (in_lines) {
+      ++line_launches;
+      return kStay;
+    }
+    if (profits && streak < kEnterAfter) ++streak;
+    if (mode == kAlways || (profits && streak >= kEnterAfter)) {
+      in_lines = true;
+      ++retiles;
+      ++line_launches;
+      return kToLines;
+    }
+    return kStay;
+  }
+  Flip set_mode(int m) {
+    mode = m;
+    streak = 0;
+    return m == kNever ? leave() : kStay;
+  }
+
+ private:
+  Flip leave() {
+    if (!in_lines) return kStay;
+    in_lines = false;
+    ++retiles;
+    return kToRows;
+  }
+};
+
+}
+}
diff --git a/metropolisengine_amd/engine.py b/metropolisengine_amd/engine.py
--- a/metropolisengine_amd/engine.py
+++ b/metropolisengine_amd/engine.py
@@ -278,6 +278,18 @@
         count = ctypes.c_uint64()
         self._check(self._lib.me_cycle_stats(self._handle, ctypes.byref(count)))
         return count.value
+
+    _STATE_FORMATS = {"never": 0, "always": 1, "auto": 2}
+
+    def set_state_format(self, mode):
+        if mode not in self._STATE_FORMATS:
+            raise ValueError("state format must be one of %s" % sorted(self._STATE_FORMATS))
+        self._check(self._lib.me_set_state_format(self._handle, self._STATE_FORMATS[mode]))
+
+    def state_format(self):
+        active, launches, retiles = ctypes.c_int32(), ctypes.c_uint64(), ctypes.c_uint64()
+        self._check(self._lib.me_state_format(self._handle, ctypes.byref(active), ctypes.byref(launches), ctypes.byref(retiles)))
+        return {"lines_active": bool(active.value), "line_launches": launches.value, "retiles": retiles.value}
 
     measure_real_system = measure
     measure_complex_system = measure
```

After: 17.64 billion. -8.2%, worse.
